# neonnnnn/sparsepoly

Measured on AMD Instinct MI355X. Metric: pcd_epochs_per_sec, higher is better.
Workload: dtype f32; 1 GPU; BASELINE configs[1]: degree=2 n_components=30 regularizer=squaredl12 solver=pcd fit_linear=True fit_lower=explicit on 1000000x100000 CSR nnz=49987865 (~50/row); schedule=colored, parallelism=single GPU, ranks=1, launcher=external, persistent_fallbacks=0

## Files before the change

sparsepoly_amd/csrc/spfm_engine_core.hip:

```cpp
#include "spfm_engine.hip.h"
#include "spfm_linear.hip.h"
#include "spfm_predict.hip.h"
#include "spfm_pbcd.hip.h"

using namespace spfm;

static thread_local std::string g_create_error;

namespace {
struct ncclUniqueId_ {
    char internal[128];
};
enum { ncclSum_ = 0 };
enum { ncclFloat64_ = 8 };
struct Rccl {
    void* lib = nullptr;
    int (*GetUniqueId)(ncclUniqueId_*) = nullptr;
    int (*CommInitRank)(ncclComm_t*, int, ncclUniqueId_, int) = nullptr;
    int (*AllReduce)(const void*, void*, size_t, int, int, ncclComm_t, hipStream_t) = nullptr;
    int (*CommDestroy)(ncclComm_t) = nullptr;
    const char* (*GetErrorString)(int) = nullptr;
    const char* (*GetLastError)(ncclComm_t) = nullptr;
    int (*GetVersion)(int*) = nullptr;
    std::string path;
// ... 1068 lines not shown
int spfm_cd_linear_epoch(spfm_handle h, double alpha, double* viol) {
    SPFM_GUARD(h);
    return h->cd_linear_epoch(alpha, viol);
}

int spfm_pcd_epoch(spfm_handle h, int order_idx, int degree, double beta, double gamma,
                   double eta, const int32_t* indices_component, int n_comp, double* viol) {
    SPFM_GUARD(h);
    return h->pcd_epoch(order_idx, degree, beta, gamma, eta, indices_component, n_comp, viol);
}

int spfm_pbcd_epoch(spfm_handle h, int order_idx, int degree, double beta, double gamma,
                    double eta, double* viol) {
    SPFM_GUARD(h);
    return h->pbcd_epoch(order_idx, degree, beta, gamma, eta, viol);
}

int spfm_host_epoch_begin(spfm_handle h, int order_idx, int degree) {
    SPFM_GUARD(h);
    return h->host_epoch_begin(order_idx, degree);
}
int spfm_host_pass_begin(spfm_handle h, int component) {
    SPFM_GUARD(h);
    return h->host_pass_begin(component);
}
int spfm_host_step_sums(spfm_handle h, int step, double* sums_out) {
    SPFM_GUARD(h);
    return h->host_step(true, step, sums_out, nullptr, nullptr);
}
int spfm_host_step_apply(spfm_handle h, int step, const double* p_new, const double* p_old) {
    SPFM_GUARD(h);
    return h->host_step(false, step, nullptr, p_new, p_old);
}
int spfm_host_epoch_end(spfm_handle h, double* viol) {
    SPFM_GUARD(h);
    return h->host_epoch_end(viol);
}

int spfm_psgd_epoch(spfm_handle h, int degree, double alpha, double beta, double gamma,
                    double eta0, int learning_rate, double power_t, int64_t batch_size,
                    const int32_t* indices_samples, int64_t n_samples, int fit_linear,
                    int64_t* it, double* sum_loss) {
    SPFM_GUARD(h);
    if (h->dist()) {
        h->err = "psgd: several ranks share this handle's communicator -- use spfm_psgd_epoch_sharded";
        return SPFM_ERR_INVALID;
    }
    return h->psgd_epoch(degree, alpha, beta, gamma, eta0, learning_rate, power_t, batch_size,
                         indices_samples, n_samples, 0, fit_linear, it, sum_loss);
}

int spfm_psgd_epoch_sharded(spfm_handle h, int degree, double alpha, double beta, double gamma,
                            double eta0, int learning_rate, double power_t, int64_t batch_size,
                            const int32_t* indices_samples, int64_t n_global, int64_t row_lo,
                            int fit_linear, int64_t* it, double* sum_loss) {
    SPFM_GUARD(h);
    return h->psgd_epoch(degree, alpha, beta, gamma, eta0, learning_rate, power_t, batch_size,
                         indices_samples, n_global, row_lo, fit_linear, it, sum_loss);
}

int spfm_comm_unique_id(char* id128) {
    if (!id128) return SPFM_ERR_INVALID;
    std::string e;
    if (!g_rccl.load(e)) {
        g_create_error = e;
        return SPFM_ERR_RUNTIME;
    }
    ncclUniqueId_ id;
    if (g_rccl.GetUniqueId(&id) != 0) {
        g_create_error = "ncclGetUniqueId failed";
        return SPFM_ERR_RUNTIME;
    }
    std::memcpy(id128, id.internal, 128);
    return SPFM_OK;
}

int spfm_comm_init(spfm_handle h, const char* id128, int n_ranks, int rank) {
    SPFM_GUARD(h);
    if (!id128 || n_ranks < 1 || rank < 0 || rank >= n_ranks) return SPFM_ERR_INVALID;
    if (!g_rccl.load(h->err)) return SPFM_ERR_RUNTIME;
    ncclUniqueId_ id;
    std::memcpy(id.internal, id128, 128);
    (void)hipStreamSynchronize(h->stream);
    const hipError_t stale = h->keep_last_error ? hipSuccess : hipGetLastError();
    int rc = g_rccl.CommInitRank(&h->comm, n_ranks, id, rank);
    if (rc != 0) {
        int ver = 0;
        if (g_rccl.GetVersion) (void)g_rccl.GetVersion(&ver);
        const char* detail = g_rccl.GetLastError ? g_rccl.GetLastError(nullptr) : nullptr;
        h->err = std::string("ncclCommInitRank: ") +
                 (g_rccl.GetErrorString ? g_rccl.GetErrorString(rc) : "error");
        if (detail && *detail) h->err += std::string(" [") + detail + "]";
        h->err += " (librccl " + std::to_string(ver) + " from " + g_rccl.path;
        h->err += std::string("; HIP last error now: ") + hipGetErrorString(hipPeekAtLastError());
        if (stale != hipSuccess)
            h->err += std::string("; cleared before the call: ") + hipGetErrorString(stale);
        h->err += "; set NCCL_DEBUG=INFO for RCCL's own log)";
        h->comm = nullptr;
        return SPFM_ERR_RUNTIME;
    }
    h->n_ranks = n_ranks;
    h->rank = rank;
    h->col_norm_reduced = false;
    h->resident_agreed.clear();
    h->clear_graphs();
    return SPFM_OK;
}

int spfm_comm_init_shm(spfm_handle h, const char* shm_name, int n_ranks, int rank) {
    SPFM_GUARD(h);
    if (!shm_name || n_ranks < 1 || n_ranks > 64 || rank < 0 || rank >= n_ranks)
        return SPFM_ERR_INVALID;
    if (h->comm || h->shm.hdr) {
        h->err = "a communicator is already attached";
        return SPFM_ERR_INVALID;
    }
    using Shm = spfm_engine::ShmComm;
    const size_t bytes = sizeof(Shm::Hdr) + sizeof(double) * Shm::kMaxDoubles * (size_t)n_ranks;
    int fd = shm_open(shm_name, O_RDWR | O_CREAT, 0600);
    if (fd < 0) {
        h->err = std::string("shm_open failed: ") + std::strerror(errno);
        return SPFM_ERR_RUNTIME;
    }
    if (ftruncate(fd, (off_t)bytes) != 0) {
        h->err = std::string("ftruncate failed: ") + std::strerror(errno);
        close(fd);
        return SPFM_ERR_RUNTIME;
    }
    void* p = mmap(nullptr, bytes, PROT_READ | PROT_WRITE, MAP_SHARED, fd, 0);
    close(fd);
    if (p == MAP_FAILED) {
        h->err = std::string("mmap failed: ") + std::strerror(errno);
        return SPFM_ERR_RUNTIME;
    }
    h->shm.hdr = reinterpret_cast<Shm::Hdr*>(p);
    h->shm.slots = reinterpret_cast<double*>(reinterpret_cast<char*>(p) + sizeof(Shm::Hdr));
    h->shm.bytes = bytes;
    h->shm.local_sense = 0;
    h->n_ranks = n_ranks;
    h->rank = rank;
    h->resident_agreed.clear();
    h->col_norm_reduced = false;
    h->clear_graphs();
    return SPFM_OK;
}

int spfm_peer_alloc(spfm_handle h, char* handle64) {
    SPFM_GUARD(h);
    if (!handle64) return SPFM_ERR_INVALID;
    if (!h->peer_own) {
        void* p = nullptr;
        hipError_t ae = hipExtMallocWithFlags(&p, sizeof(double) * spfm_engine::kPeerDoubles,
                                              hipDeviceMallocFinegrained);
        if (ae != hipSuccess) {
            (void)hipGetLastError();
            h->err = std::string("peer slab: fine-grained device memory is not available (") +
                     hipGetErrorString(ae) + "); use the per-step collective";
            return SPFM_ERR_RUNTIME;
        }
        if (hipMemsetAsync(p, 0, sizeof(double) * spfm_engine::kPeerDoubles, h->stream) != hipSuccess ||
            hipStreamSynchronize(h->stream) != hipSuccess) {
            (void)hipFree(p);
            h->err = "peer slab memset failed";
            return SPFM_ERR_RUNTIME;
        }
        h->peer_own = p;
    }
    static_assert(sizeof(hipIpcMemHandle_t) == 64, "IPC handle size");
    hipIpcMemHandle_t ih;
    hipError_t e = hipIpcGetMemHandle(&ih, h->peer_own);
    if (e != hipSuccess) {
        h->err = std::string("hipIpcGetMemHandle: ") + hipGetErrorString(e);
        return SPFM_ERR_RUNTIME;
    }
    std::memcpy(handle64, &ih, 64);
    return SPFM_OK;
}

int spfm_peer_connect(spfm_handle h, int n_ranks, int rank, const char* handles) {
    SPFM_GUARD(h);
    if (!handles || n_ranks < 2 || n_ranks > 8 || rank < 0 || rank >= n_ranks)
        return SPFM_ERR_INVALID;
    if (!h->peer_own) {
        h->err = "spfm_peer_connect: call spfm_peer_alloc first";
        return SPFM_ERR_INVALID;
    }
    if (!h->dist() || h->n_ranks != n_ranks || h->rank != rank) {
        h->err = "spfm_peer_connect: attach the communicator (spfm_comm_init[_shm]) with the "
                 "same ranks first";
        return SPFM_ERR_INVALID;
    }
    h->peer_ptr.assign((size_t)n_ranks, nullptr);
    for (int r = 0; r < n_ranks; ++r) {
        if (r == rank) {
            h->peer_ptr[(size_t)r] = h->peer_own;
            continue;
        }
        hipIpcMemHandle_t ih;
        std::memcpy(&ih, handles + (size_t)r * 64, 64);
        void* p = nullptr;
        hipError_t e = hipIpcOpenMemHandle(&p, ih, hipIpcMemLazyEnablePeerAccess);
        if (e != hipSuccess) {
            h->err = std::string("hipIpcOpenMemHandle: ") + hipGetErrorString(e);
            return SPFM_ERR_RUNTIME;
        }
        h->peer_ptr[(size_t)r] = p;
    }
    std::vector<double*> t1((size_t)n_ranks), t2((size_t)n_ranks);
    for (int r = 0; r < n_ranks; ++r) {
        t1[(size_t)r] = reinterpret_cast<double*>(h->peer_ptr[(size_t)r]) + spfm_engine::kPeerPcdOff;
        t2[(size_t)r] = reinterpret_cast<double*>(h->peer_ptr[(size_t)r]) + spfm_engine::kPeerPbOff;
    }
    if (h->upload(h->peer_tab_pcd, t1.data(), (size_t)n_ranks, 8) ||
        h->upload(h->peer_tab_pb, t2.data(), (size_t)n_ranks, 8) || h->sync()) {
        h->err = "peer table upload failed";
        return SPFM_ERR_RUNTIME;
    }
    {
        DevBuf okb;
        int ok = 0;
        h->peer_generation += 1;
        const unsigned long long word = 0x5350464d00000000ull + (unsigned)h->peer_generation;
        const unsigned long long ticks = 100ull * 1000 * 1000 * 10;
        if (okb.alloc(sizeof(int) * 4) != hipSuccess ||
            hipMemsetAsync(okb.p, 0, sizeof(int) * 4, h->stream) != hipSuccess) {
            h->err = "peer handshake: allocation failed";
            return SPFM_ERR_RUNTIME;
        }
        hipLaunchKernelGGL(peer_probe_kernel, dim3(1), dim3(kWave), 0, h->stream,
                           h->peer_tab_pcd.as<double*>(),
                           spfm_engine::kPeerProbeOff - spfm_engine::kPeerPcdOff, n_ranks, rank,
                           word, ticks, okb.as<int>());
        if (h->download(&ok, okb.p, 1) || h->sync()) {
            h->err = "peer handshake kernel failed";
            return SPFM_ERR_RUNTIME;
        }
        if (!ok) {
            h->err = "peer handshake timed out: a peer's store into this GPU's exchange slab did "
                     "not become visible to a running kernel (use the per-step collective)";
            return SPFM_ERR_RUNTIME;
        }
    }
    h->peer_ready = true;
    h->invalidate(spfm_engine::kInvSchedule | spfm_engine::kInvStreams | spfm_engine::kInvGraphs);
    return SPFM_OK;
}

int spfm_profile_enable(spfm_handle h, int on) {
    if (!h) return SPFM_ERR_INVALID;
    h->prof_on = on != 0;
    return SPFM_OK;
}

int spfm_profile_get(spfm_handle h, int which, double* ms, int64_t* launches, int64_t* nnz) {
    if (!h || which < 0 || which > 4) return SPFM_ERR_INVALID;
    if (ms) *ms = h->prof[which].ms;
    if (launches) *launches = h->prof[which].launches;
    if (nnz) *nnz = h->prof[which].nnz;
    return SPFM_OK;
}

int spfm_profile_reset(spfm_handle h) {
    if (!h) return SPFM_ERR_INVALID;
    for (auto& ps : h->prof) {
        ps.ms = 0;
        ps.launches = 0;
        ps.nnz = 0;
        ps.used = 0;
    }
    return SPFM_OK;
}

#include "spfm_options.inc.h"

int spfm_debug_prb_stamps(spfm_handle h, long long* out, int cap) {
    SPFM_GUARD(h);
    if ((h->pb_dbg & 8) && out && cap >= 8) {
        static unsigned v[16 + 4096];
        if (hipMemcpy(v, h->pb_dbgbuf.p, sizeof v, hipMemcpyDeviceToHost) != hipSuccess)
            return SPFM_ERR_RUNTIME;
        int i = 0;
        for (; i < 16 + 4096 && i < cap; ++i) out[i] = (long long)v[i];
        return i - (i % 16);
    }
    if (h->wide_stamp_on && h->wide_stamps.p && out) {
        const int nv = (int)(h->wide_stamps.bytes / sizeof(long long));
        if (cap < nv) return SPFM_ERR_INVALID;
        if (hipMemcpy(out, h->wide_stamps.p, sizeof(long long) * (size_t)nv,
                      hipMemcpyDeviceToHost) != hipSuccess)
            return SPFM_ERR_RUNTIME;
        return nv;
    }
    if (h->pb_stamp_on && (h->pb_stream_ready || h->pbr_state == 1) && out) {
        const int nv = 16 * (h->pbr_state == 1 ? h->pbr_G : h->pb_stream_G);
        if (cap < nv) return SPFM_ERR_INVALID;
        if (hipMemcpy(out, h->pb_stamps.p, sizeof(long long) * (size_t)nv,
                      hipMemcpyDeviceToHost) != hipSuccess)
            return SPFM_ERR_RUNTIME;
        return nv;
    }
    if (!h->prb_ready || !out) return SPFM_ERR_INVALID;
    const int nval = 16 * h->prb_G;
    if (cap < nval) return SPFM_ERR_INVALID;
    if (hipMemcpy(out, h->prb_stamps.p, sizeof(long long) * (size_t)nval, hipMemcpyDeviceToHost) !=
        hipSuccess)
        return SPFM_ERR_RUNTIME;
    return nval;
}

int spfm_debug_hop_latency(spfm_handle h, int partner, int rounds, double* ns_per_hop,
                           int* xcc_ids ) {
    SPFM_GUARD(h);
    if (partner < 1 || partner > 255 || rounds < 1 || rounds > (1 << 20) || !ns_per_hop)
        return SPFM_ERR_INVALID;
    DevBuf words, info;
    if (words.alloc(sizeof(unsigned long long) * 32) != hipSuccess ||
        info.alloc(sizeof(int) * 4) != hipSuccess)
        return SPFM_ERR_RUNTIME;
    hipEvent_t e0, e1;
    if (hipEventCreate(&e0) != hipSuccess || hipEventCreate(&e1) != hipSuccess)
        return SPFM_ERR_RUNTIME;
    float best = 1e30f;
    int hinfo[4] = {0, 0, 0, 0};
    for (int rep = 0; rep < 3; ++rep) {
        (void)hipMemsetAsync(words.p, 0, sizeof(unsigned long long) * 32, h->stream);
        (void)hipMemsetAsync(info.p, 0, sizeof(int) * 4, h->stream);
        (void)hipEventRecord(e0, h->stream);
        hipLaunchKernelGGL(hop_pingpong_kernel, dim3(partner + 1), dim3(kWave), 0, h->stream,
                           words.as<unsigned long long>(), rounds, partner, info.as<int>());
        (void)hipEventRecord(e1, h->stream);
        if (hipStreamSynchronize(h->stream) != hipSuccess) {
            h->err = "hop_pingpong_kernel failed";
            return SPFM_ERR_RUNTIME;
        }
        float ms = 0.f;
        (void)hipEventElapsedTime(&ms, e0, e1);
        (void)hipMemcpy(hinfo, info.p, sizeof(int) * 4, hipMemcpyDeviceToHost);
        if (hinfo[2] != 0) {
            h->err = "hop latency probe: partner workgroup did not respond";
            (void)hipEventDestroy(e0);
            (void)hipEventDestroy(e1);
            return SPFM_ERR_RUNTIME;
        }
        if (rep > 0 && ms < best) best = ms;
    }
    (void)hipEventDestroy(e0);
    (void)hipEventDestroy(e1);
    *ns_per_hop = (double)best * 1e6 / (2.0 * rounds);
    if (xcc_ids) {
        xcc_ids[0] = hinfo[0];
        xcc_ids[1] = hinfo[1];
    }
    return SPFM_OK;
}

int spfm_debug_exchange_cost(spfm_handle h, int groups, int ncols, int readers_mod, int rounds,
                             double* ns_per_round) {
    SPFM_GUARD(h);
    if (groups < 1 || groups > 256 || ncols < 1 || ncols > 64 || readers_mod == 0 ||
        rounds < 1 || rounds > (1 << 20) || !ns_per_round)
        return SPFM_ERR_INVALID;
    DevBuf slab, abortw;
    const size_t bytes = sizeof(double) * 2 * (2 * (size_t)groups + 2) * 64 * 2;
    if (slab.alloc(bytes) != hipSuccess || abortw.alloc(16) != hipSuccess) return SPFM_ERR_RUNTIME;
    PrbArgs a{};
    a.G = groups;
    a.slab = slab.as<double>();
    a.abort_flag = abortw.as<unsigned>();
    a.spin_max = 1u << 21;
    hipEvent_t e0, e1;
    if (hipEventCreate(&e0) != hipSuccess || hipEventCreate(&e1) != hipSuccess)
        return SPFM_ERR_RUNTIME;
    (void)hipFuncSetAttribute((const void*)exchange_probe_kernel,
                              hipFuncAttributeMaxDynamicSharedMemorySize, (int)h->kPrbLds);
    float best = 1e30f;
    unsigned aborted = 0;
    for (int rep = 0; rep < 3; ++rep) {
        (void)hipMemsetAsync(slab.p, 0, bytes, h->stream);
        (void)hipMemsetAsync(abortw.p, 0, 16, h->stream);
        (void)hipEventRecord(e0, h->stream);
        hipLaunchKernelGGL(exchange_probe_kernel, dim3(h->probe_xcd ? 8 * groups + 64 : groups),
                           dim3(readers_mod == -12 ? 768 : 512),
                           h->probe_xcd ? (size_t)h->probe_lds : (size_t)h->kPrbLds, h->stream, a,
                           rounds, ncols, readers_mod, h->probe_xcd);
        (void)hipEventRecord(e1, h->stream);
        if (hipStreamSynchronize(h->stream) != hipSuccess) {
            h->err = "exchange_probe_kernel failed";
            return SPFM_ERR_RUNTIME;
        }
        float ms = 0.f;
        (void)hipEventElapsedTime(&ms, e0, e1);
        (void)hipMemcpy(&aborted, abortw.p, sizeof(unsigned), hipMemcpyDeviceToHost);
        if (aborted) break;
        if (rep > 0 && ms < best) best = ms;
    }
    (void)hipEventDestroy(e0);
    (void)hipEventDestroy(e1);
    if (aborted) {
        h->err = "exchange probe timed out (workgroups not co-resident?)";
        return SPFM_ERR_RUNTIME;
    }
    *ns_per_round = (double)best * 1e6 / rounds;
    return SPFM_OK;
}

int spfm_debug_stream_probe(spfm_handle h, int64_t* bytes_out) {
    SPFM_GUARD(h);
    return h->debug_stream_probe(bytes_out);
}

int spfm_debug_write_probe(spfm_handle h, int bytes_per_record, int64_t* bytes_out) {
    SPFM_GUARD(h);
    return h->debug_write_probe(bytes_per_record, bytes_out);
}

int spfm_debug_branch_counts(spfm_handle h, unsigned* out8, int reset) {
    SPFM_GUARD(h);
    if (!out8) return SPFM_ERR_INVALID;
    if (hipStreamSynchronize(h->stream) != hipSuccess) return SPFM_ERR_RUNTIME;
    for (int i = 0; i < BR_COUNT; ++i) out8[i] = 0;
    hipError_t (*const units[])(unsigned*, int) = {
        spfm_branch_counts_pcd,       spfm_branch_counts_prb_f32,   spfm_branch_counts_prb_f64,
        spfm_branch_counts_wide,      spfm_branch_counts_pbcd,      spfm_branch_counts_pbprb_f32,
        spfm_branch_counts_pbprb_f64};
    for (auto unit : units)
        if (unit(out8, reset) != hipSuccess) return SPFM_ERR_RUNTIME;
    return SPFM_OK;
}

int spfm_set_use_graph(spfm_handle h, int on) {
    if (!h) return SPFM_ERR_INVALID;
    h->use_graph = on != 0;
    if (!on) h->clear_graphs();
    return SPFM_OK;
}

}
```

sparsepoly_amd/csrc/spfm_engine_prb.inc.h:

```cpp
#include "spfm_engine.hip.h"
#include "spfm_pcd.hip.h"

using namespace spfm;

template <typename T, int LOSS>
int spfm_engine::lin_prb(double alpha) {
    const double mu = loss == SPFM_LOSS_SQUARED ? 1.0 : (loss == SPFM_LOSS_LOGISTIC ? 0.25 : 2.0);
    int rc = ensure_prb<T>();
    if (rc) return rc;
    constexpr bool can_lr = std::is_same<T, float>::value;
    constexpr int LRV = (LOSS == LOSS_SQUARED) ? 1 : 2;
    bool relaxed = false;
    if (relax_candidate()) {
        rc = ensure_relax<T>();
        if (rc) return rc;
        relaxed = relax_state == 1;
    }
    const PrbArgs pa = relaxed ? relax_args() : prb_args();
    int lds_max = 0;
    HIPC(hipDeviceGetAttribute(&lds_max, hipDeviceAttributeMaxSharedMemoryPerBlock, device));
    const size_t lds_lr = sizeof(double) * (kPrbLdsFixed + (relaxed ? kPrbLdsCR : 0)) +
                          (size_t)pa.rows_per * 5 + 16;
    const bool use_lr = can_lr && prb_lds && lds_lr <= (size_t)lds_max && (LRV == 1 || y_pm1);
    const size_t lds_bytes = use_lr ? std::max(lds_lr, kPrbLds) : kPrbLds;
    if constexpr (can_lr) {
        if (use_lr)
            HIPC(hipFuncSetAttribute((const void*)lin_prb_kernel<T, LOSS, LRV>,
                                     hipFuncAttributeMaxDynamicSharedMemorySize,
                                     (int)lds_bytes));
    }
    HIPC(hipFuncSetAttribute((const void*)lin_prb_kernel<T, LOSS, 0>,
                             hipFuncAttributeMaxDynamicSharedMemorySize, (int)kPrbLds));
    hipLaunchKernelGGL(gather_sched_kernel, dim3(cdiv(d, 256)), dim3(256), 0, stream, d,
                       d_desc.as<ColDesc>(), w.as<double>(), prow_old.as<double>());
    HIPC(hipMemsetAsync(prb_slab.p, 0, prb_slab.bytes, stream));
    if (relaxed) HIPC(hipMemsetAsync(r_cslab.p, 0, r_cslab.bytes, stream));
    {
        int prc = peer_clear(kPeerPcdOff, kPeerPbOff);
        if (prc) return prc;
    }
    prof_begin(4, nnz);
    bool launched = false;
    auto launch_cr = [&](auto lr_tag, size_t lds) -> int {
        constexpr int LRc = decltype(lr_tag)::value;
        auto* fn = lin_prb_kernel<T, LOSS, LRc, false, true>;
        HIPC(hipFuncSetAttribute((const void*)fn, hipFuncAttributeMaxDynamicSharedMemorySize,
                                 (int)lds));
        if (!resident_ok((const void*)fn, kPrbThreads, lds, prb_G)) return kNotResident;
        hipLaunchKernelGGL(fn, dim3(launch_groups(prb_G)), dim3(kPrbThreads), lds, stream, pa,
                           r_eval.as<T>(), yy.as<T>(), prow_old.as<double>(),
                           prb_cn.as<double>(), w.as<double>(), alpha, mu,
                           prb_viol.as<double>());
        return SPFM_OK;
    };
    auto launch = [&](auto lr_tag, auto mg_tag, size_t lds) -> int {
        constexpr int LRc = decltype(lr_tag)::value;
        constexpr bool MGc = decltype(mg_tag)::value;
        HIPC(hipFuncSetAttribute((const void*)lin_prb_kernel<T, LOSS, LRc, MGc>,
                                 hipFuncAttributeMaxDynamicSharedMemorySize, (int)lds));
        if (!resident_ok((const void*)lin_prb_kernel<T, LOSS, LRc, MGc>, kPrbThreads, lds, prb_G))
            return kNotResident;
        hipLaunchKernelGGL((lin_prb_kernel<T, LOSS, LRc, MGc>), dim3(launch_groups(prb_G)),
                           dim3(kPrbThreads),
                           lds, stream, pa, prb_eval.as<T>(), yy.as<T>(),
                           prow_old.as<double>(), prb_cn.as<double>(), w.as<double>(), alpha,
                           mu, prb_viol.as<double>());
        return SPFM_OK;
    };
    int lrc = SPFM_OK;
    if (relaxed) {
        launched = true;
        bool done = false;
        if constexpr (can_lr) {
            if (use_lr) {
                lrc = launch_cr(std::integral_constant<int, LRV>{}, lds_bytes);
                done = true;
            }
        }
        if (!done) lrc = launch_cr(std::integral_constant<int, 0>{}, kPrbLds);
    }
    if constexpr (can_lr) {
        if (use_lr && !launched) {
            lrc = pa.n_ranks > 1
                      ? launch(std::integral_constant<int, LRV>{}, std::true_type{}, lds_bytes)
                      : launch(std::integral_constant<int, LRV>{}, std::false_type{}, lds_bytes);
            launched = true;
        }
    }
    if (!launched)
        lrc = pa.n_ranks > 1
                  ? launch(std::integral_constant<int, 0>{}, std::true_type{}, kPrbLds)
                  : launch(std::integral_constant<int, 0>{}, std::false_type{}, kPrbLds);
    if (lrc == kNotResident) prof_cancel(4, nnz);
    if (lrc) return lrc;
    prof_end(4);
    hipLaunchKernelGGL(fold_viol_kernel, dim3(cdiv(d, 256)), dim3(256), 0, stream, d,
                       d_desc.as<ColDesc>(), prb_viol.as<double>(), viol_col.as<double>());
    HIPC(hipGetLastError());
    return SPFM_OK;
}

template <typename T>
int spfm_engine::lin_prb_loss(double alpha) {
    switch (loss) {
        case SPFM_LOSS_SQUARED: return lin_prb<T, LOSS_SQUARED>(alpha);
        case SPFM_LOSS_SQUARED_HINGE: return lin_prb<T, LOSS_SQUARED_HINGE>(alpha);
        default: return lin_prb<T, LOSS_LOGISTIC>(alpha);
    }
}

template <typename T>
int spfm_engine::ensure_prb() {
    if (prb_ready) return SPFM_OK;
    int ncu = 0;
    HIPC(hipDeviceGetAttribute(&ncu, hipDeviceAttributeMultiprocessorCount, device));
    if (prb_G > ncu) prb_G = ncu;
    if (prb_G < 1) prb_G = 1;
    const int nb_ = n_batches();
    std::unique_lock<std::mutex> cache_lock;
    std::string ckey;
    bool hit = false;
    if (scache) {
        ckey = fkey("prb", {}, {(int64_t)sched_hash, prb_G, prb_long, (int64_t)sizeof(T), nb_});
        cache_lock = std::unique_lock<std::mutex>(scache->mu);
        for (auto& e : scache->prb)
            if (e->key == ckey) {
                prb_sp.share(e->sp);
                prb_erow.share(e->erow);
                prb_eval.share(e->eval);
                prb_lmask.share(e->lmask);
                prb_has_long = e->has_long;
                stream_device_used = 2;
                hit = true;
                break;
            }
    }
    if (!hit) {
        int rc = build_prb_stream<T>(nb_);
        if (rc) return rc;
        if (scache) {
            auto e = std::make_unique<StreamCache::Prb>();
            e->key = ckey;
            e->sp.share(prb_sp);
            e->erow.share(prb_erow);
            e->eval.share(prb_eval);
            e->lmask.share(prb_lmask);
            e->has_long = prb_has_long;
            scache->prb.insert(scache->prb.begin(), std::move(e));
            if (scache->prb.size() > StreamCache::kKeep) scache->prb.pop_back();
        }
    }
    if (cache_lock.owns_lock()) cache_lock.unlock();
    HIPC(prb_slab.alloc(sizeof(double) * 2 * ((size_t)prb_G + 1) * 64 * 2));
    HIPC(prb_abort.alloc(sizeof(unsigned) * 4));
    HIPC(prow_old.alloc(sizeof(double) * (size_t)d));
    HIPC(prb_viol.alloc(sizeof(double) * (size_t)d));
    HIPC(prb_cn.alloc(sizeof(double) * (size_t)d));
    HIPC(prb_stamps.alloc(sizeof(long long) * 16 * (size_t)prb_G));
    HIPC(hipMemsetAsync(prb_stamps.p, 0, prb_stamps.bytes, stream));
    HIPC(hipMemsetAsync(prb_abort.p, 0, sizeof(unsigned) * 4, stream));
    HIPC(hipMemsetAsync(prb_slab.p, 0, prb_slab.bytes, stream));
    hipLaunchKernelGGL(gather_sched_kernel, dim3(cdiv(d, 256)), dim3(256), 0, stream, d,
                       d_desc.as<ColDesc>(), col_norm.as<double>(), prb_cn.as<double>());
    HIPC(hipGetLastError());
    HIPC(hipStreamSynchronize(stream));
    prb_ready = true;
    return SPFM_OK;
}

template <typename T>
int spfm_engine::build_prb_stream(int nb_) {
    const size_t nsp = (size_t)prb_G * nb_ * 65 + 1;
    DevBuf d_src;
    HIPC(d_src.alloc(sizeof(int32_t) * (size_t)(nnz > 0 ? nnz : 1)));
    HIPC(prb_sp.alloc(sizeof(int32_t) * nsp));
    HIPC(prb_lmask.alloc(sizeof(uint32_t) * (size_t)prb_G * nb_ * 2));
    stream_device_used = 0;
    if (stream_device && nnz >= (1 << 20)) {
        int hl = 0;
        const hipError_t e = device_rowblock_stream(
            n, d, nnz, prb_G, nb_, prb_long, d_order.as<int32_t>(), d_bptr.as<int32_t>(),
            cptr.as<int64_t>(), cidx.as<int32_t>(), nullptr, prb_sp.as<int32_t>(),
            d_src.as<int32_t>(), prb_lmask.as<uint32_t>(), &hl, nullptr, stream);
        if (e == hipSuccess) {
            prb_has_long = hl;
            stream_device_used = 1;
        } else {
            (void)hipGetLastError();
        }
    }
    std::vector<int32_t> sp, src;
    std::vector<uint32_t> lmask;
    if (!stream_device_used) {
        build_rowblock_stream(n, h_cptr.data(), h_cidx.data(), order, batch_ptr, prb_G,
                              prb_long, sp, src, lmask, nullptr);
        prb_has_long = 0;
        for (uint32_t m : lmask) prb_has_long |= (m != 0u);
        SPFM_TRY(upload_to(prb_lmask.p, lmask.data(), lmask.size()));
    }
    HIPC(prb_erow.alloc(sizeof(int32_t) * (size_t)(nnz > 0 ? nnz : 1)));
    HIPC(prb_eval.alloc(sizeof(T) * (size_t)(nnz > 0 ? nnz : 1)));
    if (!stream_device_used)
        SPFM_TRY(upload_to(prb_sp.p, sp.data(), sp.size()));
    if (nnz > 0) {
        if (!stream_device_used)
            SPFM_TRY(upload_to(d_src.p, src.data(), (size_t)nnz));
        hipLaunchKernelGGL((prb_gather_kernel<T>), dim3(cdiv(nnz, 256)), dim3(256), 0, stream,
                           nnz, d_src.as<int32_t>(), cidx.as<int32_t>(), cval.as<T>(),
                           prb_erow.as<int32_t>(), prb_eval.as<T>());
        HIPC(hipGetLastError());
    }
    HIPC(hipStreamSynchronize(stream));
    return SPFM_OK;
}

template <typename T>
int spfm_engine::ensure_relax() {
    if (relax_state != 0) return SPFM_OK;
    relax_state = -1;
    int rc = ensure_prb<T>();
    if (rc) return rc;
    std::vector<int32_t> cf_ptr, cf_row, cf_qq, sp, src;
    std::vector<int64_t> cf_ia, cf_ib;
    std::vector<int16_t> clist;
    std::vector<uint8_t> skip;
    std::vector<uint32_t> lmask;
    schedule_relax(n, d, h_cptr.data(), h_cidx.data(), order.data(), 64, 64, r_batch_ptr, cf_ptr,
                   cf_row, cf_qq, cf_ia, cf_ib, clist, skip);
    const int nbr = (int)r_batch_ptr.size() - 1;
    if ((double)nbr > 0.6 * (double)n_batches()) return SPFM_OK;
    DevBuf d_src;
    HIPC(r_bptr.alloc(sizeof(int32_t) * r_batch_ptr.size()));
    SPFM_TRY(upload_to(r_bptr.p, r_batch_ptr.data(), r_batch_ptr.size()));
    const size_t nsp_r = (size_t)prb_G * nbr * 65 + 1;
    bool dev_stream = false;
    size_t ne = 0;
    if (stream_device && nnz >= (1 << 20)) {
        DevBuf d_skip;
        HIPC(d_skip.alloc((size_t)nnz));
        SPFM_TRY(upload_to(d_skip.p, skip.data(), (size_t)nnz));
        HIPC(d_src.alloc(sizeof(int32_t) * (size_t)nnz));
        HIPC(r_sp.alloc(sizeof(int32_t) * nsp_r));
        HIPC(r_lmask.alloc(sizeof(uint32_t) * (size_t)prb_G * nbr * 2));
        int hl = 0;
        int64_t tot = 0;
        const hipError_t e = device_rowblock_stream(
            n, d, nnz, prb_G, nbr, prb_long, d_order.as<int32_t>(), r_bptr.as<int32_t>(),
            cptr.as<int64_t>(), cidx.as<int32_t>(), d_skip.as<uint8_t>(), r_sp.as<int32_t>(),
            d_src.as<int32_t>(), r_lmask.as<uint32_t>(), &hl, &tot, stream);
        if (e == hipSuccess) {
            relax_has_long = hl;
            ne = (size_t)tot;
            dev_stream = true;
        } else {
            (void)hipGetLastError();
        }
    }
    if (!dev_stream) {
        build_rowblock_stream(n, h_cptr.data(), h_cidx.data(), order, r_batch_ptr, prb_G,
                              prb_long, sp, src, lmask, skip.data());
        relax_has_long = 0;
        for (uint32_t m : lmask) relax_has_long |= (m != 0u);
        ne = src.size();
    }
    const size_t ncf = cf_row.size();
    std::vector<PrbConf<T>> hcf(ncf ? ncf : 1);
    {
        std::vector<T> hv((size_t)(nnz > 0 ? nnz : 1));
        SPFM_TRY(download(hv.data(), cval.p, (size_t)nnz));
        HIPC(hipStreamSynchronize(stream));
        for (size_t c = 0; c < ncf; ++c) {
            hcf[c].row = cf_row[c];
            hcf[c].qq = cf_qq[c];
            hcf[c].xa = hv[(size_t)cf_ia[c]];
            hcf[c].xb = hv[(size_t)cf_ib[c]];
        }
    }
    if (!dev_stream) {
        HIPC(d_src.alloc(sizeof(int32_t) * (ne ? ne : 1)));
        HIPC(r_sp.alloc(sizeof(int32_t) * sp.size()));
        HIPC(r_lmask.alloc(sizeof(uint32_t) * lmask.size()));
    }
    HIPC(r_erow.alloc(sizeof(int32_t) * (ne ? ne : 1)));
    HIPC(r_eval.alloc(sizeof(T) * (ne ? ne : 1)));
    HIPC(r_cfptr.alloc(sizeof(int32_t) * cf_ptr.size()));
    HIPC(r_cf.alloc(sizeof(PrbConf<T>) * hcf.size()));
    HIPC(r_clist.alloc(sizeof(int16_t) * clist.size() + 16));
    HIPC(r_cslab.alloc(sizeof(double) * 2 * 64 * 8));
    if (!dev_stream) {
        SPFM_TRY(upload_to(r_sp.p, sp.data(), sp.size()));
        SPFM_TRY(upload_to(r_lmask.p, lmask.data(), lmask.size()));
    }
    SPFM_TRY(upload_to(r_cfptr.p, cf_ptr.data(), cf_ptr.size()));
    SPFM_TRY(upload_to(r_cf.p, hcf.data(), hcf.size()));
    SPFM_TRY(upload_to(r_clist.p, clist.data(), clist.size()));
    if (ne > 0) {
        if (!dev_stream)
            SPFM_TRY(upload_to(d_src.p, src.data(), ne));
        hipLaunchKernelGGL((prb_gather_kernel<T>), dim3(cdiv((int64_t)ne, 256)), dim3(256), 0,
                           stream, (int64_t)ne, d_src.as<int32_t>(), cidx.as<int32_t>(),
                           cval.as<T>(), r_erow.as<int32_t>(), r_eval.as<T>());
        HIPC(hipGetLastError());
    }
    HIPC(hipStreamSynchronize(stream));
    relax_state = 1;
    return SPFM_OK;
}

template <typename T, int M, int LOSS>
int spfm_engine::pcd_pass_prb(int order_idx, double beta, double gamma, double eta) {
    const double mu = loss == SPFM_LOSS_SQUARED ? 1.0 : (loss == SPFM_LOSS_LOGISTIC ? 0.25 : 2.0);
    int rc = ensure_prb<T>();
    if (rc) return rc;
    double* Po = P.as<double>() + (size_t)order_idx * k * d;
    Ctl* c = ctl.as<Ctl>();
    double* cb = cache.as<double>();
    constexpr bool can_lr = std::is_same<T, float>::value && Kind<M>::AS <= 2;
    constexpr int LRV = (LOSS == LOSS_SQUARED) ? 1 : 2;
    constexpr bool can_stamp = std::is_same<T, float>::value && M == 2 && LOSS == LOSS_SQUARED;
    constexpr bool can_stamp3 = std::is_same<T, float>::value && M == 3 && LOSS == LOSS_SQUARED;
    if (prb_stamp_on && !((can_stamp && prb_lds) || (can_stamp3 && !prb_lds)))
        FAIL(SPFM_ERR_UNSUPPORTED,
             "prb_stamps: built for float storage, squared loss and degree 2 with prb_lds=1 "
             "or degree 3 with prb_lds=0 only");
    bool relaxed = false;
    if constexpr (M == 2 || M == 3) {
        if (relax_candidate() && !prb_stamp_on) {
            rc = ensure_relax<T>();
            if (rc) return rc;
            relaxed = relax_state == 1;
        }
    }
    PrbArgs pa = relaxed ? relax_args() : prb_args();
    constexpr bool can_pk = std::is_same<T, float>::value && M == 3;
    bool packed = false;
    if (prb_stamp_on && pa.n_ranks > 1)
        FAIL(SPFM_ERR_UNSUPPORTED,
             "prb_stamps: the timer instantiation has no cross-GPU stage (single rank only)");
    int lds_max = 0;
    HIPC(hipDeviceGetAttribute(&lds_max, hipDeviceAttributeMaxSharedMemoryPerBlock, device));
    const size_t lds_lr = sizeof(double) * (kPrbLdsFixed + (relaxed ? kPrbLdsCR : 0)) +
                          (size_t)pa.rows_per * (4 * Kind<M>::AS + (LRV == 1 ? 4 : 5)) + 16;
    const bool use_lr = can_lr && prb_lds && lds_lr <= (size_t)lds_max &&
                        (LRV == 1 || y_pm1);
    const size_t lds_bytes = use_lr ? std::max(lds_lr, kPrbLds) : kPrbLds;
    prb_lds_active = use_lr ? LRV : 0;
    hipLaunchKernelGGL(begin_pass_kernel, dim3(1), dim3(64), 0, stream, c,
                       comp_order.as<int32_t>(), lams.as<double>());
    if (reg != SPFM_REG_L1) {
        hipLaunchKernelGGL((pcd_compute_cache_kernel<M>), dim3(kCacheBlocks), dim3(kBlock), 0,
                           stream, c, Po, d, reg, partial.as<double>());
        hipLaunchKernelGGL((pcd_cache_combine_kernel<M>), dim3(1), dim3(64), 0, stream, reg,
                           kCacheBlocks, partial.as<double>(), cb);
    }
    hipLaunchKernelGGL(snapshot_row_kernel, dim3(cdiv(d, 256)), dim3(256), 0, stream, c, Po, d,
                       d_desc.as<ColDesc>(), prow_old.as<double>());
    HIPC(hipMemsetAsync(prb_slab.p, 0, prb_slab.bytes, stream));
    if (relaxed) HIPC(hipMemsetAsync(r_cslab.p, 0, r_cslab.bytes, stream));
    if constexpr (can_pk) {
        if (!use_lr && !prb_stamp_on && prb_pack) {
            HIPC(prb_rec.alloc(sizeof(float) * 4 * (size_t)n));
            pa.rec = prb_rec.p;
            hipLaunchKernelGGL(prb_pack3_kernel, dim3(cdiv(n, 256)), dim3(256), 0, stream, c, n,
                               (size_t)n * 2, yy.as<float>(), A.as<float>(),
                               prb_rec.as<float4>());
            packed = true;
        }
    }
    {
        int prc = peer_clear(kPeerPcdOff, kPeerPbOff);
        if (prc) return prc;
    }
    prof_begin(0, nnz);
    auto go = [&](auto lr_tag, auto stamp_tag, auto reg_tag) -> int {
        constexpr int LRc = decltype(lr_tag)::value;
        constexpr bool STc = decltype(stamp_tag)::value;
        constexpr int RGc = decltype(reg_tag)::value;
        const size_t lds = (LRc == 1 || LRc == 2) ? lds_bytes : kPrbLds;
        auto launch = [&](auto mg_tag) -> int {
            constexpr bool MGc = decltype(mg_tag)::value;
            HIPC(hipFuncSetAttribute(
                (const void*)pcd_prb_kernel<T, M, LOSS, LRc, STc, RGc, MGc>,
                hipFuncAttributeMaxDynamicSharedMemorySize, (int)lds));
            if (!resident_ok((const void*)pcd_prb_kernel<T, M, LOSS, LRc, STc, RGc, MGc>,
                             kPrbThreads, lds, prb_G))
                return kNotResident;
            hipLaunchKernelGGL((pcd_prb_kernel<T, M, LOSS, LRc, STc, RGc, MGc>),
                               dim3(launch_groups(prb_G)), dim3(kPrbThreads), lds, stream, c, pa, prb_eval.as<T>(),
                               A.as<T>(), (size_t)n * Kind<M>::AS, yy.as<T>(),
                               prow_old.as<double>(), Po, d, reg, cb, mu, beta, gamma, eta,
                               prb_viol.as<double>());
            return SPFM_OK;
        };
        if constexpr (STc) {
            return launch(std::false_type{});
        } else {
            return pa.n_ranks > 1 ? launch(std::true_type{}) : launch(std::false_type{});
        }
    };
    using std::integral_constant;
    int lrc = SPFM_OK;
    bool launched = false;
    if constexpr (M == 2 || M == 3) {
        if (relaxed) {
            auto launch_cr = [&](auto lr_tag) -> int {
                constexpr int LRc = decltype(lr_tag)::value;
                const size_t lds = (LRc == 1 || LRc == 2) ? lds_bytes : kPrbLds;
                auto* fn = pcd_prb_kernel<T, M, LOSS, LRc, false, -1, false, true>;
                HIPC(hipFuncSetAttribute((const void*)fn,
                                         hipFuncAttributeMaxDynamicSharedMemorySize, (int)lds));
                if (!resident_ok((const void*)fn, kPrbThreads, lds, prb_G)) return kNotResident;
                hipLaunchKernelGGL(fn, dim3(launch_groups(prb_G)), dim3(kPrbThreads), lds, stream,
                                   c, pa, r_eval.as<T>(), A.as<T>(), (size_t)n * Kind<M>::AS,
                                   yy.as<T>(), prow_old.as<double>(), Po, d, reg, cb, mu, beta,
                                   gamma, eta, prb_viol.as<double>());
                return SPFM_OK;
            };
            launched = true;
            bool done = false;
            if constexpr (can_lr) {
                if (use_lr) {
                    lrc = launch_cr(integral_constant<int, LRV>{});
                    done = true;
                }
            }
            if constexpr (can_pk) {
                if (!done && packed) {
                    lrc = launch_cr(integral_constant<int, 3>{});
                    done = true;
                }
            }
            if (!done) lrc = launch_cr(integral_constant<int, 0>{});
        }
    }
    if constexpr (can_lr) {
        if (use_lr && !launched) {
            launched = true;
            if constexpr (can_stamp) {
                if (prb_stamp_on)
                    lrc = go(integral_constant<int, LRV>{}, std::true_type{},
                             integral_constant<int, -1>{});
            }
            if (!prb_stamp_on) {
                if (reg == SPFM_REG_L1)
                    lrc = go(integral_constant<int, LRV>{}, std::false_type{},
                             integral_constant<int, REG_L1>{});
                else if (reg == SPFM_REG_OMEGATI)
                    lrc = go(integral_constant<int, LRV>{}, std::false_type{},
                             integral_constant<int, REG_OMEGATI>{});
                else if constexpr (M == 2)
                    lrc = go(integral_constant<int, LRV>{}, std::false_type{},
                             integral_constant<int, REG_SQL12>{});
                else
                    lrc = go(integral_constant<int, LRV>{}, std::false_type{},
                             integral_constant<int, -1>{});
            }
        }
    }
    if constexpr (can_pk) {
        if (!launched && packed) {
            launched = true;
// ... 61 lines not shown
```

sparsepoly_amd/csrc/spfm_pcd.hip.h:

```cpp
#pragma once
#include "spfm_common.hip.h"

namespace spfm {


template <typename T, int M>
__global__ __launch_bounds__(kBlock) void pcd_precompute_all_kernel(
    int64_t n, int k, const int64_t* __restrict__ rptr, const int32_t* __restrict__ ridx,
    const T* __restrict__ rval, const double* __restrict__ Pt, T* __restrict__ A_all) {
    constexpr int R = 32;
    constexpr int RP = R + 1;
    extern __shared__ __attribute__((aligned(16))) unsigned char pre_lds[];
    T* tile = reinterpret_cast<T*>(pre_lds);
    const int tid = threadIdx.x, lane = tid & 63, wave = tid >> 6;
    for (int64_t tile0 = (int64_t)blockIdx.x * R; tile0 < n; tile0 += (int64_t)gridDim.x * R) {
        for (int s0 = 0; s0 < k; s0 += kWave) {
            const int s = s0 + lane;
            const bool sv = s < k;
            for (int r = wave; r < R; r += kBlock / kWave) {
                const int64_t i = tile0 + r;
                if (i >= n) break;
                constexpr int NA = (M == 0) ? 2 : M;
                double a[NA];
                a[0] = 1.0;
// ... 373 lines not shown
            double r;
            {
                const double dc2 = c10 - a_i;
                const double m0 = p_i - s_i * (c20 - dc2 * a_i);
                r = (m0 > 0) ? m0 : 0.0;
            }
            bool fixed = false;
            unsigned long long negl = 0ull;
            double be1 = 0.0, be2 = 0.0;
            for (int round = 0; round < 8 && !fixed; ++round) {
                const double d1 = r - a_i;
                double al1 = 1.0;
                be1 = d1;
                affine_scan_inclusive(al1, be1, lane);
                const double c1b = affine_before(al1, be1, c10, lane);
                const double dc2 = c1b - a_i;
                double al2 = 1.0;
                be2 = dc2 * d1;
                affine_scan_inclusive(al2, be2, lane);
                const double c2b = affine_before(al2, be2, c20, lane);
                const double dc3 = c2b - dc2 * a_i;
                const double m = p_i - s_i * dc3;
                const double rn = (m > 0) ? m : 0.0;
                negl = __ballot(act && ((__double2hiint(dc2) | __double2hiint(dc3)) < 0));
                fixed = __ballot(__double_as_longlong(rn) != __double_as_longlong(r)) == 0ull;
                r = rn;
            }
            if (fixed && negl == 0ull) {
                cache[1] = c10 + readlane_d(be1, 63);
                cache[2] = c20 + readlane_d(be2, 63);
                return sg * (act ? r : 0.0);
            }
        }
        if constexpr (M > 2) {
            {
                const bool in = lane <= last;
                double* my = sc + lane * 4;
                my[0] = in ? ab : 0.0;
                my[1] = in ? st : 0.0;
                my[2] = in ? apin : 0.0;
            }
            asm volatile("s_waitcnt lgkmcnt(0)" ::: "memory");
            double c[M + 1];
#pragma unroll
            for (int t = 0; t <= M; ++t) c[t] = cache[t];
            unsigned neg = 0u;
            const int nblk = (last + 4) >> 2;
            auto sweep = [&](auto clip_tag) __attribute__((always_inline)) {
                constexpr bool CLIP = decltype(clip_tag)::value;
                double na[4], ns[4], np[4];
#pragma unroll
                for (int u = 0; u < 4; ++u) {
                    na[u] = sc[u * 4];
                    ns[u] = sc[u * 4 + 1];
                    np[u] = sc[u * 4 + 2];
                }
                for (int blk = 0; blk < nblk; ++blk) {
                    double ca[4], cs[4], cp[4];
                    double* nx = sc + (blk + 1) * 16;
#pragma unroll
                    for (int u = 0; u < 4; ++u) {
                        ca[u] = na[u];
                        cs[u] = ns[u];
                        cp[u] = np[u];
                        na[u] = nx[u * 4];
                        ns[u] = nx[u * 4 + 1];
                        np[u] = nx[u * 4 + 2];
                    }
#pragma unroll
                    for (int u = 0; u < 4; ++u) {
                        const double ai = ca[u], si = cs[u], pi = cp[u];
                        double dc[M + 2];
                        dc[1] = 1.0;
#pragma unroll
                        for (int deg = 2; deg <= M; ++deg) {
                            double v = c[deg - 1];
                            v -= dc[deg - 1] * ai;
                            if constexpr (CLIP) {
                                dc[deg] = (v < 0) ? 0.0 : v;
                            } else {
                                neg |= (unsigned)__double2hiint(v);
                                dc[deg] = v;
                            }
                        }
                        const double m = pi - si * dc[M];
                        const double r = (m > 0) ? m : 0.0;
#pragma unroll
                        for (int deg = 1; deg < M; ++deg) c[deg] = dc[deg + 1] + dc[deg] * r;
                        sc[(blk * 4 + u) * 4 + 3] = r;
                    }
                }
            };
            if (lane == 0) sweep(std::false_type{});
            if (__builtin_amdgcn_readfirstlane((int)neg) < 0) {
                count_branch(BR_OMEGATI_CLIP, lane);
#pragma unroll
                for (int t = 0; t <= M; ++t) c[t] = cache[t];
                if (lane == 0) sweep(std::true_type{});
            }
#pragma unroll
            for (int t = 1; t < M; ++t) cache[t] = readlane_d(c[t], 0);
            asm volatile("s_waitcnt lgkmcnt(0)" ::: "memory");
            mine = (lane <= last) ? sc[lane * 4 + 3] : 0.0;
        }
        return sg * mine;
    }
}


template <int M>
__device__ __forceinline__ double pcd_chain_waves(int reg, int lane, int wave, int ncols, bool valid,
                                                  double p_old, double g, double h, double lam,
                                                  double mu, double beta, double gamma, double eta,
                                                  double (&cache)[M + 1], double* sh_map,
                                                  int* sh_bad) {
    static_assert(M == 2, "wide steps: degree 2");
    double pin = 0.0, st = 0.0;
    if (valid) {
        double inv = h * mu;
        inv += beta;
        double upd = g * lam;
        upd += beta * p_old;
        const double rinv = recip_nr(inv);
        upd *= rinv;
        pin = p_old - eta * upd;
        st = (eta * gamma) * rinv;
    }
    if (reg == REG_L1) {
        const double sg = (pin > 0) ? 1.0 : ((pin < 0) ? -1.0 : 0.0);
        const double m = fabs(pin) - st;
        return sg * (m > 0.0 ? m : 0.0);
    }
    const bool sq = reg == REG_SQL12;
    const int nw = (ncols + 63) >> 6;
    const int last = min(64, ncols - 64 * wave) - 1;
    const bool act = valid && lane <= last;
    const double ab = fabs(p_old);
    double app, tt, sg;
    if (sq) {
        const double rden = recip_nr(1 + 2 * st);
        const double pp = pin * rden;
        app = fabs(pp);
        tt = (2 * st) * rden;
        sg = (pp > 0) ? 1.0 : -1.0;
    } else {
        app = fabs(pin);
        tt = st;
        sg = (pin > 0) ? 1.0 : -1.0;
    }
    const int ci = sq ? 0 : 1;
    const double c0 = cache[ci];
    bool pos = sq ? true : ((c0 - ab) >= 0);
    bool nz = (app - tt * (pos ? (c0 - ab) : 0.0)) > 0;
    double al = 1.0, be = 0.0, m = 0.0;
    auto scan = [&]() __attribute__((always_inline)) {
        if (!act) {
            al = 1.0;
            be = 0.0;
        } else if (!pos) {
            al = 0.0;
            be = app;
        } else if (nz) {
            al = 1.0 - tt;
            be = app - al * ab;
        } else {
            al = 1.0;
            be = -ab;
        }
        affine_scan_inclusive(al, be, lane);
    };
    scan();
    bool dirty = true;
    double mA[8], mB[8];
#pragma unroll
    for (int w = 0; w < 8; ++w) {
        mA[w] = 1.0;
        mB[w] = 0.0;
    }
    for (int gr = 0; gr < 3 * kWave; ++gr) {
        if (dirty && lane == 0) {
            sh_map[wave * 2] = last >= 0 ? readlane_d(al, last >= 0 ? last : 0) : 1.0;
            sh_map[wave * 2 + 1] = last >= 0 ? readlane_d(be, last >= 0 ? last : 0) : 0.0;
        }
        if (wave == 0 && lane == 0) {
            if (gr == 0) sh_bad[0] = sh_bad[1] = sh_bad[2] = 0;
            else sh_bad[(gr + 1) % 3] = 0;
        }
        asm volatile("s_waitcnt lgkmcnt(0)\n\ts_barrier" ::: "memory");
#pragma unroll
        for (int w = 0; w < 8; ++w) {
            mA[w] = sh_map[w * 2];
            mB[w] = sh_map[w * 2 + 1];
        }
        double c_in = c0;
#pragma unroll
        for (int w = 0; w < 7; ++w)
            if (w < wave) c_in = mA[w] * c_in + mB[w];
        bool changed = false;
        for (int lr = 0; lr <= kWave; ++lr) {
            const double cb = affine_before(al, be, c_in, lane);
            const double v = cb - ab;
            const bool pos2 = sq ? true : !(v < 0);
            const double u = pos2 ? v : 0.0;
            m = sq ? fma(-tt, u, app) : (app - tt * u);
            const bool nz2 = m > 0;
            const unsigned long long bad =
                __ballot(act && ((pos2 != pos) || (pos2 && (nz2 != nz))));
            pos = pos2;
            nz = nz2;
            if (bad == 0ull) break;
            changed = true;
            scan();
        }
        dirty = changed;
        if (changed && lane == 0) sh_bad[gr % 3] = 1;
        asm volatile("s_waitcnt lgkmcnt(0)\n\ts_barrier" ::: "memory");
        if (sh_bad[gr % 3] == 0) break;
    }
    if (!sq && __ballot(act && !pos) != 0ull) count_branch(BR_OMEGATI_CLIP, lane);
    double c_end = c0;
#pragma unroll
    for (int w = 0; w < 8; ++w)
        if (w < nw) c_end = mA[w] * c_end + mB[w];
    cache[ci] = c_end;
    const double r = sq ? ((act && nz) ? m : 0.0) : (act ? ((m > 0) ? m : 0.0) : 0.0);
    return sg * r;
}

template <int M>
__global__ __launch_bounds__(kWave) void pcd_chain_kernel(
    const Ctl* __restrict__ ctl, const ColDesc* __restrict__ desc, int ncols,
    double* __restrict__ P, int d, const double* __restrict__ part,
    const double* __restrict__ pold, int reg, const double* __restrict__ cache_in,
    double* __restrict__ cache_out, double mu, double beta, double gamma, double eta,
    double* __restrict__ delta, double* __restrict__ viol_col) {
    __shared__ double sh_chain[(kWave + 4) * 4];
    const int lane = threadIdx.x;
    const double lam = ctl->lam;
    double* ps = P + (size_t)ctl->s * d;
    double cache[M + 1];
#pragma unroll
    for (int t = 0; t <= M; ++t) cache[t] = cache_in[t];
    for (int base = 0; base < ncols; base += kWave) {
        const int q = base + lane;
        const bool valid = q < ncols;
        const int cnt = min(kWave, ncols - base);
        double p_old = 0.0, g = 0.0, h = 0.0;
        int j = 0;
        if (valid) {
            j = desc[q].j;
            p_old = pold[q];
            g = part[2 * q];
            h = part[2 * q + 1];
        }
        const double res =
            pcd_chain_lanes<M>(reg, lane, cnt - 1, valid, p_old, g, h, lam, mu, beta, gamma, eta,
                               cache, sh_chain);
        if (valid) {
            const double dl = p_old - res;
            ps[j] = res;
            delta[q] = dl;
            viol_col[j] += fabs(dl);
        }
    }
    if (lane == 0) {
#pragma unroll
        for (int t = 0; t <= M; ++t) cache_out[t] = cache[t];
    }
}


template <typename T, int M>
__device__ __forceinline__ void pcd_sync_entry(size_t i, double x, double p_old, double upd,
                                               double lam, T* __restrict__ A,
                                               T* __restrict__ yy) {
    if constexpr (M == 0) {
        const double a0 = (double)A[i];
        double yh = (double)yy[2 * i];
        yh -= lam * a0;
        double a1 = a0 / (1.0 + x * p_old);
        a1 *= 1.0 + x * (p_old - upd);
        yh += lam * a1;
        A[i] = (T)a1;
        yy[2 * i] = (T)yh;
        return;
    }
    double dprev = x;
#pragma unroll
    for (int t = 1; t < M; ++t) {
        const size_t at = i * (M - 1) + (t - 1);
        const double a = (double)A[at];
        const double dcur = x * (a - p_old * dprev);
        A[at] = (T)(a - upd * dprev);
        dprev = dcur;
    }
    const double yh = (double)yy[2 * i];
    yy[2 * i] = (T)(yh - lam * upd * dprev);
}

template <typename T, int M>
__device__ __forceinline__ void pcd_sync_entry_lds(int il, double x, double p_old, double upd,
                                                   double lam, T* lds_a, T* lds_r) {
    constexpr int AS = Kind<M>::AS;
    double yh = (double)lds_r[il];
    if constexpr (M == 0) {
        const double a0 = (double)lds_a[il];
        yh -= lam * a0;
        double a1 = a0 / (1.0 + x * p_old);
        a1 *= 1.0 + x * (p_old - upd);
        yh += lam * a1;
        lds_a[il] = (T)a1;
        lds_r[il] = (T)yh;
    } else {
        double dprev = x;
#pragma unroll
        for (int t = 0; t < AS; ++t) {
            const double a = (double)lds_a[il * AS + t];
            const double dcur = x * (a - p_old * dprev);
            lds_a[il * AS + t] = (T)(a - upd * dprev);
            dprev = dcur;
        }
        lds_r[il] = (T)(yh - lam * upd * dprev);
    }
}

template <typename T, int M>
__global__ __launch_bounds__(kBlock) void pcd_sync_kernel(
    const Ctl* __restrict__ ctl, const ColDesc* __restrict__ desc,
    const int32_t* __restrict__ cidx, const T* __restrict__ cval, T* __restrict__ A_all,
    size_t a_stride, T* __restrict__ yy , const double* __restrict__ delta,
    const double* __restrict__ pold) {
    const int q = blockIdx.x;
    const double upd = delta[q];
    if (upd == 0.0) return;
    T* __restrict__ A = A_all + (size_t)ctl->s * a_stride;
    const double p_old = pold[q];
    const double lam = ctl->lam;
    const ColDesc cd = desc[q];
    const int64_t b = cd.start, e = cd.start + cd.len;
    for (int64_t ii = b + threadIdx.x; ii < e; ii += kBlock)
        pcd_sync_entry<T, M>((size_t)cidx[ii], (double)cval[ii], p_old, upd, lam, A, yy);
}

template <typename T, int M>
__global__ __launch_bounds__(kBlock) void pcd_chain_sync_kernel(
    const Ctl* __restrict__ ctl, const ColDesc* __restrict__ desc, int ncols,
    double* __restrict__ P, int d, const double* __restrict__ part,
    const double* __restrict__ pold, int reg, const double* __restrict__ cache_in,
    double* __restrict__ cache_out, double mu, double beta, double gamma, double eta,
    const int32_t* __restrict__ cidx, const T* __restrict__ cval, T* __restrict__ A_all,
    size_t a_stride, T* __restrict__ yy, double* __restrict__ viol_col) {
    __shared__ double sh[2];
    __shared__ double sh_chain[(kWave + 4) * 4];
    T* __restrict__ A = A_all + (size_t)ctl->s * a_stride;
    constexpr int PF = 2;
    const int q = blockIdx.x;
    const int tid = threadIdx.x, lane = tid & 63, wave = tid >> 6;
    const ColDesc cd = desc[q];
    const double lam = ctl->lam;
    int ri[PF];
    double rx[PF];
    bool rv[PF];
#pragma unroll
    for (int u = 0; u < PF; ++u) {
        const int off = tid + u * kBlock;
        rv[u] = off < cd.len;
        ri[u] = rv[u] ? cidx[cd.start + off] : 0;
        rx[u] = rv[u] ? (double)cval[cd.start + off] : 0.0;
    }
    if (wave == 0) {
        const bool valid = lane < ncols;
        double p_old = 0.0, g = 0.0, h = 0.0;
        if (valid) {
            p_old = pold[lane];
            g = part[2 * lane];
            h = part[2 * lane + 1];
        }
        double cache[M + 1];
#pragma unroll
        for (int t = 0; t <= M; ++t) cache[t] = cache_in[t];
        const double res = pcd_chain_lanes<M>(reg, lane, q, valid, p_old, g, h, lam, mu, beta,
                                              gamma, eta, cache, sh_chain);
        if (lane == q) {
            const double dl = p_old - res;
            P[(size_t)ctl->s * d + cd.j] = res;
            viol_col[cd.j] += fabs(dl);
            sh[0] = dl;
            sh[1] = p_old;
        }
        if (q == ncols - 1 && lane == 0) {
#pragma unroll
            for (int t = 0; t <= M; ++t) cache_out[t] = cache[t];
        }
    }
    __syncthreads();
    const double upd = sh[0];
    if (upd == 0.0) return;
    const double p_old = sh[1];
#pragma unroll
    for (int u = 0; u < PF; ++u)
        if (rv[u]) pcd_sync_entry<T, M>((size_t)ri[u], rx[u], p_old, upd, lam, A, yy);
    for (int64_t ii = cd.start + tid + PF * kBlock; ii < cd.start + cd.len; ii += kBlock)
        pcd_sync_entry<T, M>((size_t)cidx[ii], (double)cval[ii], p_old, upd, lam, A, yy);
}


}
```

sparsepoly_amd/csrc/spfm_prb.hip.h:

```cpp
#pragma once
#include "spfm_common.hip.h"
#include "spfm_pcd.hip.h"

namespace spfm {


struct PrbArgs {
    int G;
    int nb;
    const int32_t* bptr;
    const ColDesc* desc;
    const int32_t* sp;
    const uint32_t* lmask;
    int has_long;
    const int32_t* erow;
    double* slab;
    int rows_per;
    int n_rows;
    unsigned* abort_flag;
    unsigned spin_max;
    long long* stamps;
    int n_ranks, rank;
    double* const* xslab;
    const int32_t* cf_ptr;
    const void* cf;
    const int16_t* clist;
    double* cslab;
    void* rec;
};

template <typename T>
struct __attribute__((aligned(8))) PrbConf {
    int32_t row;
    int32_t qq;
    T xa, xb;
};


__device__ __forceinline__ void st_agent(double* p, double v) {
    __hip_atomic_store(reinterpret_cast<unsigned long long*>(p),
                       (unsigned long long)__double_as_longlong(v), __ATOMIC_RELAXED,
                       __HIP_MEMORY_SCOPE_AGENT);
}
__device__ __forceinline__ double ld_agent(const double* p) {
    const unsigned long long u =
        __hip_atomic_load(reinterpret_cast<const unsigned long long*>(p), __ATOMIC_RELAXED,
                          __HIP_MEMORY_SCOPE_AGENT);
    return __longlong_as_double((long long)u);
}

__device__ __forceinline__ unsigned long long prb_tag(int b) {
    return (unsigned long long)(((b >> 1) % 3) + 1);
}
__device__ __forceinline__ void prb_store_granule(double* p, double v, unsigned long long tag) {
    const unsigned long long u =
        ((unsigned long long)__double_as_longlong(v) & ~3ull) | tag;
    __hip_atomic_store(reinterpret_cast<unsigned long long*>(p), u, __ATOMIC_RELAXED,
                       __HIP_MEMORY_SCOPE_AGENT);
}
__device__ __forceinline__ unsigned long long prb_load_granule(const double* p) {
    return __hip_atomic_load(reinterpret_cast<const unsigned long long*>(p), __ATOMIC_RELAXED,
                             __HIP_MEMORY_SCOPE_AGENT);
}

__device__ __forceinline__ void prb_store_granule_l2(double* p, double v, unsigned long long tag) {
    const unsigned long long u =
        ((unsigned long long)__double_as_longlong(v) & ~3ull) | tag;
    asm volatile("global_store_dwordx2 %0, %1, off" ::"v"(p), "v"(u) : "memory");
}

__device__ __forceinline__ void prb_store_granule_sys(double* p, double v, unsigned long long tag) {
    const unsigned long long u =
        ((unsigned long long)__double_as_longlong(v) & ~3ull) | tag;
    __hip_atomic_store(reinterpret_cast<unsigned long long*>(p), u, __ATOMIC_RELAXED,
                       __HIP_MEMORY_SCOPE_SYSTEM);
}
__device__ __forceinline__ unsigned long long prb_load_granule_sys(const double* p) {
    return __hip_atomic_load(reinterpret_cast<const unsigned long long*>(p), __ATOMIC_RELAXED,
                             __HIP_MEMORY_SCOPE_SYSTEM);
}

template <int NV>
__device__ __forceinline__ bool prb_cross_gpu(const PrbArgs& a, int g, int b, int lane,
                                              double* tot) {
    const unsigned long long tag = prb_tag(b);
    const size_t par_off = (size_t)(b & 1) * a.n_ranks * 64 * 2;
    if (g == 0) {
        for (int rr = 0; rr < a.n_ranks; ++rr) {
            double* dst = a.xslab[rr] + par_off + ((size_t)a.rank * 64 + lane) * 2;
#pragma unroll
            for (int v = 0; v < NV; ++v) prb_store_granule_sys(dst + v, tot[v], tag);
        }
    }
    const double* mine = a.xslab[a.rank] + par_off + (size_t)lane * 2;
    double acc[NV];
#pragma unroll
    for (int v = 0; v < NV; ++v) acc[v] = 0.0;
    for (int rr = 0; rr < a.n_ranks; ++rr) {
        unsigned long long t[NV];
        unsigned spins = 0;
        for (;;) {
            bool all = true;
#pragma unroll
            for (int v = 0; v < NV; ++v) {
                t[v] = prb_load_granule_sys(mine + (size_t)rr * 64 * 2 + v);
                all = all && ((t[v] & 3ull) == tag);
            }
            if (all) break;
            if ((++spins & 63u) == 0) {
                if (__hip_atomic_load(a.abort_flag, __ATOMIC_RELAXED, __HIP_MEMORY_SCOPE_AGENT) ||
                    spins > a.spin_max) {
                    __hip_atomic_store(a.abort_flag, 1u, __ATOMIC_RELAXED,
                                       __HIP_MEMORY_SCOPE_AGENT);
                    return false;
                }
            }
        }
#pragma unroll
        for (int v = 0; v < NV; ++v) acc[v] += __longlong_as_double((long long)(t[v] & ~3ull));
    }
#pragma unroll
    for (int v = 0; v < NV; ++v) tot[v] = acc[v];
    return true;
}

typedef unsigned __attribute__((ext_vector_type(4))) prb_u4;

__device__ __forceinline__ void prb_load_pairs8(const double* const* p, prb_u4* r) {
    asm volatile(
        "global_load_dwordx4 %0, %8, off sc1\n\t"
        "global_load_dwordx4 %1, %9, off sc1\n\t"
        "global_load_dwordx4 %2, %10, off sc1\n\t"
        "global_load_dwordx4 %3, %11, off sc1\n\t"
        "global_load_dwordx4 %4, %12, off sc1\n\t"
        "global_load_dwordx4 %5, %13, off sc1\n\t"
        "global_load_dwordx4 %6, %14, off sc1\n\t"
        "global_load_dwordx4 %7, %15, off sc1\n\t"
        "s_waitcnt vmcnt(0)"
        : "=&v"(r[0]), "=&v"(r[1]), "=&v"(r[2]), "=&v"(r[3]), "=&v"(r[4]), "=&v"(r[5]),
          "=&v"(r[6]), "=&v"(r[7])
        : "v"(p[0]), "v"(p[1]), "v"(p[2]), "v"(p[3]), "v"(p[4]), "v"(p[5]), "v"(p[6]), "v"(p[7])
        : "memory");
}

template <int NV>
__device__ __forceinline__ bool prb_collect_quarter(const PrbArgs& a, int b, int w, int lane,
                                                    int ncols, double* out ,
                                                    int nparts = 4) {
    const double* slab = a.slab + (size_t)(b & 1) * a.G * 64 * 2;
    const unsigned long long tag = prb_tag(b);
    const int g0 = (a.G * w) / nparts, g1 = (a.G * (w + 1)) / nparts;
    double tot[NV];
#pragma unroll
    for (int v = 0; v < NV; ++v) tot[v] = 0.0;
    bool ok = true;
    if (lane < ncols) {
        const double* sl = slab + (size_t)lane * 2;
        constexpr int GU = 8;
        for (int gg = g0; gg < g1; gg += GU) {
            unsigned long long t[GU][NV];
            unsigned spins = 0;
            for (;;) {
                bool all = true;
                if constexpr (NV == 2) {
                    const double* ptr[GU];
                    prb_u4 r[GU];
#pragma unroll
                    for (int u = 0; u < GU; ++u)
                        ptr[u] = sl + (size_t)((gg + u < g1) ? gg + u : g1 - 1) * 128;
                    prb_load_pairs8(ptr, r);
#pragma unroll
                    for (int u = 0; u < GU; ++u) {
                        t[u][0] = ((unsigned long long)r[u].y << 32) | r[u].x;
                        t[u][1] = ((unsigned long long)r[u].w << 32) | r[u].z;
                        all = all && ((t[u][0] & 3ull) == tag) && ((t[u][1] & 3ull) == tag);
                    }
                } else {
#pragma unroll
                    for (int u = 0; u < GU; ++u)
#pragma unroll
                        for (int v = 0; v < NV; ++v) {
                            const bool in = gg + u < g1;
                            t[u][v] = in ? prb_load_granule(sl + (size_t)(gg + u) * 128 + v) : tag;
                            all = all && ((t[u][v] & 3ull) == tag);
                        }
                }
                if (all) break;
                if ((++spins & 63u) == 0) {
                    if (__hip_atomic_load(a.abort_flag, __ATOMIC_RELAXED,
                                          __HIP_MEMORY_SCOPE_AGENT) ||
                        spins > a.spin_max) {
                        __hip_atomic_store(a.abort_flag, 1u, __ATOMIC_RELAXED,
                                           __HIP_MEMORY_SCOPE_AGENT);
                        ok = false;
                        break;
                    }
                }
            }
            if (!ok) break;
#pragma unroll
            for (int u = 0; u < GU; ++u)
#pragma unroll
                for (int v = 0; v < NV; ++v)
                    if (gg + u < g1) tot[v] += __longlong_as_double((long long)(t[u][v] & ~3ull));
        }
    }
#pragma unroll
    for (int v = 0; v < NV; ++v) out[((size_t)w * 64 + lane) * 2 + v] = tot[v];
    return ok;
}

constexpr int PRB_PF = 4;
constexpr int kPrbLong = 48;
template <typename T>
struct PrbEntries {
    int e0, e1;
    int row[PRB_PF];
    T x[PRB_PF];
};

__device__ __forceinline__ void prb_load_sp(const PrbArgs& a, int g, int b, int slot, int ncols,
                                            int& e0, int& e1, unsigned long long& lmask) {
    e0 = 0;
    e1 = 0;
    lmask = 0ull;
    const int32_t* spb = a.sp + ((size_t)g * a.nb + b) * 65;
    if (a.has_long) {
        const uint32_t* lm = a.lmask + ((size_t)g * a.nb + b) * 2;
        lmask = ((unsigned long long)lm[1] << 32) | (unsigned long long)lm[0];
        if (slot < ncols && !((lmask >> slot) & 1ull)) {
            e0 = spb[slot];
            e1 = spb[slot + 1];
        }
    } else if (slot < ncols) {
        e0 = spb[slot];
        e1 = spb[slot + 1];
    }
}

__device__ __forceinline__ int nth_set_bit(unsigned long long m, int q) {
    for (int t = 0; t < q; ++t) m &= m - 1;
    return __builtin_ctzll(m);
}

template <typename T>
__device__ __forceinline__ void prb_load_entries(const PrbArgs& a, const T* __restrict__ eval,
                                                 int e0, int e1, int sub, PrbEntries<T>& en,
                                                 int pad_row = 0) {
    en.e0 = e0;
    en.e1 = e1;
#pragma unroll
    for (int u = 0; u < PRB_PF; ++u) {
        const int e = e0 + sub + 4 * u;
        const bool v = e < e1;
        en.row[u] = v ? a.erow[e] : pad_row;
        en.x[u] = v ? eval[e] : (T)0;
    }
}

constexpr int kPrbThreads = 512;
constexpr int kPrbParts = 8;
constexpr int kPrbLdsFixed = 2560;

template <int NV>
__device__ __forceinline__ bool prb_poll(const PrbArgs& a, const double* p, unsigned long long tag,
                                         double* out);

__device__ __forceinline__ void pcd_sync_entry_rec(size_t i, double x, double p_old, double upd,
                                                   double lam, float4* __restrict__ rec) {
    const float4 r = rec[i];
    const double a1 = (double)r.z, a2 = (double)r.w;
    const double d1 = x * (a1 - p_old * x);
    const double d2 = x * (a2 - p_old * d1);
    float4 o;
    o.x = (float)((double)r.x - lam * upd * d2);
    o.y = r.y;
    o.z = (float)(a1 - upd * x);
    o.w = (float)(a2 - upd * d1);
    rec[i] = o;
}

static __global__ void prb_pack3_kernel(const Ctl* __restrict__ ctl, int64_t n, size_t a_stride,
                                 const float* __restrict__ yy, const float* __restrict__ A_all,
                                 float4* __restrict__ rec) {
    const int64_t i = (int64_t)blockIdx.x * blockDim.x + threadIdx.x;
    if (i < n) {
        const float* A = A_all + (size_t)ctl->s * a_stride;
        float4 r;
        r.x = yy[2 * i];
        r.y = yy[2 * i + 1];
        r.z = A[2 * i];
        r.w = A[2 * i + 1];
        rec[i] = r;
    }
}
static __global__ void prb_unpack3_kernel(const Ctl* __restrict__ ctl, int64_t n, size_t a_stride,
                                   const float4* __restrict__ rec, float* __restrict__ yy,
                                   float* __restrict__ A_all) {
    const int64_t i = (int64_t)blockIdx.x * blockDim.x + threadIdx.x;
    if (i < n) {
        float* A = A_all + (size_t)ctl->s * a_stride;
        const float4 r = rec[i];
        yy[2 * i] = r.x;
        A[2 * i] = r.z;
        A[2 * i + 1] = r.w;
    }
}

constexpr int kPrbLdsCR = 256;
template <typename T, int M, int LOSS, int LR, bool STAMP = false, int REGC = -1, bool MG = false,
          bool CR = false>
__global__ __launch_bounds__(kPrbThreads) void pcd_prb_kernel(
    const Ctl* __restrict__ ctl, PrbArgs a, const T* __restrict__ eval, T* __restrict__ A_all,
    size_t a_stride, T* __restrict__ yy, const double* __restrict__ pold_sched,
    double* __restrict__ P, int d, int reg, const double* __restrict__ cache_in, double mu,
    double beta, double gamma, double eta, double* __restrict__ viol_pos) {
    T* __restrict__ A = A_all + (size_t)ctl->s * a_stride;
    extern __shared__ __attribute__((aligned(16))) double dyn_lds[];
    double* sh_delta = dyn_lds + 128;
    double* sh_pold = dyn_lds + 192;
    double* sh_chain = dyn_lds + 256;
    double* sh_quart = dyn_lds + 1536;
    int* sh_ok = reinterpret_cast<int*>(dyn_lds + 768);
    int* sh_go = reinterpret_cast<int*>(dyn_lds + 770);
    const typename Vec2<T>::type* yy2 = reinterpret_cast<const typename Vec2<T>::type*>(yy);
    const int g = blockIdx.x;
    const int tid = threadIdx.x, lane = tid & 63, wave = tid >> 6;
    const bool control = wave == 0;
    const bool worker = wave >= 1 && wave <= 4;
    const int part = worker ? wave - 1 : (control ? 4 : wave);
    const int wt = tid - 64;
    const int slot = worker ? (wt >> 2) : 64, sub = wt & 3;
    const int s = ctl->s;
    const double lam = ctl->lam;
    double* ps = P + (size_t)s * d;
    double cache[M + 1];
#pragma unroll
    for (int t = 0; t <= M; ++t) cache[t] = cache_in[t];

    double* sh_long = dyn_lds + 1024;
    constexpr bool LDSR = (LR == 1 || LR == 2);
    constexpr bool PK = (LR == 3);
    static_assert(!LDSR || (Kind<M>::AS <= 2 && sizeof(T) == 4 &&
                            (LR == 2 || LOSS == LOSS_SQUARED)),
                  "LDS-resident rows: float storage, one or two cache values per row");
    static_assert(!PK || (sizeof(T) == 4 && Kind<M>::AS == 2),
                  "packed row records: float storage, two cache values per row");
    float4* __restrict__ rec = reinterpret_cast<float4*>(a.rec);
    constexpr int AS = Kind<M>::AS;
    static_assert(!CR || (M >= 2 && !MG && !STAMP), "relaxed runs: degree >= 2, single GPU");
    constexpr int CSN = 2 + Kind<M>::AS;
    constexpr int CSS = 8;
    const int row0 = LDSR ? g * a.rows_per : 0;
    double* sh_ce = dyn_lds + kPrbLdsFixed;
    double* sh_cv = sh_ce + 128;
    T* lds_a = reinterpret_cast<T*>(dyn_lds + kPrbLdsFixed + (CR ? kPrbLdsCR : 0));
    T* lds_r = lds_a + (size_t)a.rows_per * AS;
    unsigned char* lds_s = reinterpret_cast<unsigned char*>(lds_r + a.rows_per);
    if constexpr (LDSR) {
        const int nr = min(a.rows_per, a.n_rows - row0);
        for (int il = tid; il < nr; il += kPrbThreads) {
            const typename Vec2<T>::type yv = yy2[(size_t)(row0 + il)];
#pragma unroll
            for (int t = 0; t < AS; ++t) lds_a[il * AS + t] = A[(size_t)(row0 + il) * AS + t];
            if constexpr (LR == 1) {
                lds_r[il] = (T)((double)yv.x - (double)yv.y);
            } else {
                lds_r[il] = yv.x;
                lds_s[il] = yv.y > (T)0 ? 1 : 0;
            }
        }
        __syncthreads();
    }
    PrbEntries<T> cur, nxt;
    int c0 = a.bptr[0], c1 = a.bptr[1];
    int c2 = (a.nb > 1) ? a.bptr[2] : c1;
    int c3 = (a.nb > 2) ? a.bptr[3] : c2;
    unsigned long long lm0 = 0ull, lm1 = 0ull;
    {
        int e0, e1;
        prb_load_sp(a, g, 0, slot, c1 - c0, e0, e1, lm0);
        prb_load_entries<T>(a, eval, e0, e1, sub, cur, row0);
    }
    int ne0 = 0, ne1 = 0;
    if (a.nb > 1) prb_load_sp(a, g, 1, slot, c2 - c1, ne0, ne1, lm1);
    double p_slot = (slot < c1 - c0) ? pold_sched[c0 + slot] : 0.0;
    if (tid == 0) {
        *sh_ok = 1;
        *sh_go = 0;
    }
    int cp0 = 0, cp1 = 0, cp2 = 0, cp3 = 0;
    PrbConf<T> cfc, cfn;
    cfc.row = cfn.row = 0;
    cfc.qq = cfn.qq = 0;
    cfc.xa = cfc.xb = cfn.xa = cfn.xb = (T)0;
    prb_u4 clq = {~0u, ~0u, ~0u, ~0u}, clqn = {~0u, ~0u, ~0u, ~0u};
    if constexpr (CR) {
        if (control) {
            const PrbConf<T>* cfa = reinterpret_cast<const PrbConf<T>*>(a.cf);
            cp0 = a.cf_ptr[0];
            cp1 = a.cf_ptr[min(1, a.nb)];
            cp2 = a.cf_ptr[min(2, a.nb)];
            cp3 = a.cf_ptr[min(3, a.nb)];
            if (lane < cp1 - cp0) cfc = cfa[cp0 + lane];
            if (lane < c1 - c0)
                clq = reinterpret_cast<const prb_u4*>(a.clist)[c0 + lane];
        }
    }
    long long acc[8] = {0, 0, 0, 0, 0, 0, 0, 0};
    long long tprev = STAMP ? clock64() : 0;
#define PRB_STAMP(k)                        \
    if constexpr (STAMP) {                  \
        if (tid == 0) {                     \
            const long long tn = clock64(); \
            acc[k] += tn - tprev;           \
            tprev = tn;                     \
        }                                   \
    }
#define PRB_HSTAMP(k)                       \
    if constexpr (STAMP) {                  \
        if (tid == 320) {                   \
            const long long tn = clock64(); \
            acc[k] += tn - tprev;           \
            tprev = tn;                     \
        }                                   \
    }
#define PRB_WSTAMP(k)                       \
    if constexpr (STAMP) {                  \
        if (tid == 64) {                    \
            const long long tn = clock64(); \
            acc[k] += tn - tprev;           \
            tprev = tn;                     \
        }                                   \
    }

    for (int b = 0; b < a.nb; ++b) {
        const int ncols = c1 - c0;
        const int c4 = (b + 4 <= a.nb) ? a.bptr[b + 4] : c3;
        __builtin_amdgcn_s_waitcnt(0x0F70);
        double av[PRB_PF][AS];
        double yh[PRB_PF], yt[PRB_PF], dlast[PRB_PF];
        double pl = 0.0;
        int jl = 0;
        double cst[CSN];
#pragma unroll
        for (int t = 0; t < CSN; ++t) cst[t] = 0.0;
        if (control) {
            if (lane < ncols) {
                pl = pold_sched[c0 + lane];
                if (g == 0) jl = a.desc[c0 + lane].j;
            }
            if constexpr (CR) {
                const int nc = cp1 - cp0, ncw = max(nc, cp3 - cp2);
                const unsigned long long ctag = prb_tag(b);
                double* cs = a.cslab + ((size_t)(b & 1) * 64 + lane) * CSS;
                if (lane < nc) {
                    const int i = cfc.row;
                    if (i / a.rows_per == g) {
                        double st[CSN];
                        if constexpr (LDSR) {
                            st[0] = (double)lds_r[i - row0];
                            st[1] = (LR == 1) ? 0.0 : (lds_s[i - row0] ? 1.0 : -1.0);
#pragma unroll
                            for (int t = 0; t < AS; ++t) st[2 + t] = (double)lds_a[(i - row0) * AS + t];
                        } else if constexpr (PK) {
                            const float4 r = rec[(size_t)i];
                            st[0] = (double)r.x;
                            st[1] = (double)r.y;
                            st[2] = (double)r.z;
                            st[2 + AS - 1] = (double)r.w;
                        } else {
                            const typename Vec2<T>::type yv = yy2[(size_t)i];
                            st[0] = (double)yv.x;
                            st[1] = (double)yv.y;
#pragma unroll
                            for (int t = 0; t < AS; ++t) st[2 + t] = (double)A[(size_t)i * AS + t];
                        }
#pragma unroll
                        for (int t = 0; t < CSN; ++t) prb_store_granule(cs + t, st[t], ctag);
                    }
                } else if (lane < ncw && (lane % a.G) == g) {
#pragma unroll
                    for (int t = 0; t < CSN; ++t) prb_store_granule(cs + t, 0.0, ctag);
                }
            }
        } else if (worker) {
#pragma unroll
            for (int u = 0; u < PRB_PF; ++u) {
                if constexpr (LDSR) {
                    const int il = cur.row[u] - row0;
                    yh[u] = (double)lds_r[il];
                    yt[u] = (LR == 1) ? 0.0 : (lds_s[il] ? 1.0 : -1.0);
#pragma unroll
                    for (int t = 0; t < AS; ++t) av[u][t] = (double)lds_a[il * AS + t];
                } else if constexpr (PK) {
                    const float4 r = rec[(size_t)cur.row[u]];
                    yh[u] = (double)r.x;
                    yt[u] = (double)r.y;
                    av[u][0] = (double)r.z;
                    av[u][AS - 1] = (double)r.w;
                } else {
                    const size_t i = (size_t)cur.row[u];
                    const typename Vec2<T>::type yv = yy2[i];
                    yh[u] = (double)yv.x;
                    yt[u] = (double)yv.y;
#pragma unroll
                    for (int t = 0; t < AS; ++t) av[u][t] = (double)A[i * AS + t];
                }
            }
            double ag = 0.0, ah = 0.0;
#pragma unroll
            for (int u = 0; u < PRB_PF; ++u) {
                const double dprev = grad_factor<M>(av[u], (double)cur.x[u], p_slot);
                dlast[u] = dprev;
                const double dl = dloss_dev(LOSS, yh[u], yt[u]);
                const bool v = cur.e0 + sub + 4 * u < cur.e1;
                ag += v ? dl * dprev : 0.0;
                ah += v ? dprev * dprev : 0.0;
            }
            for (int e = cur.e0 + sub + 4 * PRB_PF; e < cur.e1; e += 4) {
                const int i = a.erow[e];
                const double x = (double)eval[e];
                double a1[AS], y0, y1;
                if constexpr (LDSR) {
                    y0 = (double)lds_r[i - row0];
                    y1 = (LR == 1) ? 0.0 : (lds_s[i - row0] ? 1.0 : -1.0);
#pragma unroll
                    for (int t = 0; t < AS; ++t) a1[t] = (double)lds_a[(i - row0) * AS + t];
                } else if constexpr (PK) {
                    const float4 r = rec[(size_t)i];
                    y0 = (double)r.x;
                    y1 = (double)r.y;
                    a1[0] = (double)r.z;
                    a1[AS - 1] = (double)r.w;
                } else {
                    const typename Vec2<T>::type yv = yy2[i];
                    y0 = (double)yv.x;
                    y1 = (double)yv.y;
#pragma unroll
                    for (int t = 0; t < AS; ++t) a1[t] = (double)A[(size_t)i * AS + t];
                }
                const double dprev = grad_factor<M>(a1, x, p_slot);
                ag += dloss_dev(LOSS, y0, y1) * dprev;
                ah += dprev * dprev;
            }
            ag += dpp_move_d<0xB1, 0xf>(0.0, ag);
            ah += dpp_move_d<0xB1, 0xf>(0.0, ah);
            ag += dpp_move_d<0x4E, 0xf>(0.0, ag);
            ah += dpp_move_d<0x4E, 0xf>(0.0, ah);
            PRB_WSTAMP(0)
            if (sub == 0 && !((lm0 >> slot) & 1ull)) {
                double* sl = a.slab + (size_t)(b & 1) * a.G * 64 * 2 + ((size_t)g * 64 + slot) * 2;
                const unsigned long long tag = prb_tag(b);
                prb_store_granule(sl, ag, tag);
                prb_store_granule(sl + 1, ah, tag);
            }
        }
        const unsigned long long lmu =
            ((unsigned long long)__builtin_amdgcn_readfirstlane((int)(lm0 >> 32)) << 32) |
            (unsigned)__builtin_amdgcn_readfirstlane((int)lm0);
        if (lmu != 0ull) {
            const int32_t* spb = a.sp + ((size_t)g * a.nb + b) * 65;
            int qi = 0;
            for (unsigned long long mm = lmu; mm != 0ull; mm &= mm - 1, ++qi) {
                const int q = __builtin_ctzll(mm);
                if (worker) {
                    const int le0 = spb[q], le1 = spb[q + 1];
                    const double pq = pold_sched[c0 + q];
                    double lg = 0.0, lh = 0.0;
                    for (int e = le0 + wt; e < le1; e += 256) {
                        const int i = a.erow[e];
                        const double x = (double)eval[e];
                        double a1[Kind<M>::AS], y0, y1;
                        if constexpr (LDSR) {
                            y0 = (double)lds_r[i - row0];
                            y1 = (LR == 1) ? 0.0 : (lds_s[i - row0] ? 1.0 : -1.0);
#pragma unroll
                            for (int t = 0; t < Kind<M>::AS; ++t)
                                a1[t] = (double)lds_a[(i - row0) * Kind<M>::AS + t];
                        } else if constexpr (PK) {
                            const float4 r = rec[(size_t)i];
                            y0 = (double)r.x;
                            y1 = (double)r.y;
                            a1[0] = (double)r.z;
                            a1[Kind<M>::AS - 1] = (double)r.w;
                        } else {
                            const typename Vec2<T>::type yv = yy2[i];
                            y0 = (double)yv.x;
                            y1 = (double)yv.y;
#pragma unroll
                            for (int t = 0; t < Kind<M>::AS; ++t)
                                a1[t] = (double)A[(size_t)i * Kind<M>::AS + t];
                        }
                        const double dprev = grad_factor<M>(a1, x, pq);
                        lg += dloss_dev(LOSS, y0, y1) * dprev;
                        lh += dprev * dprev;
                    }
                    lg = wave_sum(lg);
                    lh = wave_sum(lh);
                    if (lane == 0) {
                        sh_long[(qi * 4 + (wave - 1)) * 2] = lg;
                        sh_long[(qi * 4 + (wave - 1)) * 2 + 1] = lh;
                    }
                }
            }
            __syncthreads();
            if (worker && wt < qi) {
                const int q = nth_set_bit(lmu, wt);
                double tg = 0.0, th = 0.0;
                for (int w4 = 0; w4 < 4; ++w4) {
                    tg += sh_long[(wt * 4 + w4) * 2];
                    th += sh_long[(wt * 4 + w4) * 2 + 1];
                }
                double* sl = a.slab + (size_t)(b & 1) * a.G * 64 * 2 + ((size_t)g * 64 + q) * 2;
                const unsigned long long tag = prb_tag(b);
                prb_store_granule(sl, tg, tag);
                prb_store_granule(sl + 1, th, tag);
            }
        }
        PRB_STAMP(0)
        double p_next = 0.0;
        int n2e0 = 0, n2e1 = 0;
        unsigned long long lm2 = 0ull;
        if (b + 2 < a.nb) prb_load_sp(a, g, b + 2, slot, c3 - c2, n2e0, n2e1, lm2);
        if (worker) {
            PRB_WSTAMP(1)
            if (tid == 64 + 255)
                __hip_atomic_store(sh_go, b + 1, __ATOMIC_RELAXED, __HIP_MEMORY_SCOPE_WORKGROUP);
            if (LDSR && b + 1 < a.nb) {
                prb_load_entries<T>(a, eval, ne0, ne1, sub, nxt, row0);
                if (slot < c2 - c1) p_next = pold_sched[c1 + slot];
            }
            {
                const bool ok =
                    prb_collect_quarter<2>(a, b, part, lane, ncols, sh_quart, kPrbParts);
                if (!ok) *sh_ok = 0;
            }
            PRB_WSTAMP(2)
            if (!LDSR && b + 1 < a.nb) {
                prb_load_entries<T>(a, eval, ne0, ne1, sub, nxt, row0);
                if (slot < c2 - c1) p_next = pold_sched[c1 + slot];
            }
        } else {
            unsigned spins = 0;
            while (__hip_atomic_load(sh_go, __ATOMIC_RELAXED, __HIP_MEMORY_SCOPE_WORKGROUP) <
                       b + 1 &&
                   ++spins < (1u << 24))
                __builtin_amdgcn_s_sleep(1);
            PRB_HSTAMP(1)
            const bool ok = prb_collect_quarter<2>(a, b, part, lane, ncols, sh_quart, kPrbParts);
            if (!ok) *sh_ok = 0;
            PRB_HSTAMP(2)
            if constexpr (CR) {
                if (control) {
                    if (lane < cp1 - cp0) {
                        if (!prb_poll<CSN>(a, a.cslab + ((size_t)(b & 1) * 64 + lane) * CSS,
                                           prb_tag(b), cst))
                            *sh_ok = 0;
                    }
                    const PrbConf<T>* cfa = reinterpret_cast<const PrbConf<T>*>(a.cf);
                    if (lane < cp2 - cp1) cfn = cfa[cp1 + lane];
                    clqn = prb_u4{~0u, ~0u, ~0u, ~0u};
                    if (lane < c2 - c1) clqn = reinterpret_cast<const prb_u4*>(a.clist)[c1 + lane];
                }
            }
        }
        PRB_WSTAMP(3)
        asm volatile("s_waitcnt lgkmcnt(0)\n\ts_barrier" ::: "memory");
        if (!*sh_ok) break;
        PRB_STAMP(3)
        PRB_HSTAMP(7)
        PRB_WSTAMP(4)
        if (control) {
            double tot[2];
#pragma unroll
            for (int v = 0; v < 2; ++v) {
                tot[v] = sh_quart[lane * 2 + v];
#pragma unroll
                for (int w = 1; w < kPrbParts; ++w) tot[v] += sh_quart[(w * 64 + lane) * 2 + v];
            }
            if constexpr (MG) {
                if (!prb_cross_gpu<2>(a, g, b, lane, tot)) *sh_ok = 0;
            }
            const bool valid = lane < ncols;
            bool serial = false;
            if constexpr (CR) serial = (cp1 - cp0) > 0;
            if (!serial) {
                const double res = pcd_chain_lanes<M>(REGC >= 0 ? REGC : reg, lane, ncols - 1, valid,
                                                      pl, tot[0], tot[1], lam, mu, beta, gamma, eta,
                                                      cache, sh_chain);
                const double dl = valid ? (pl - res) : 0.0;
                sh_delta[lane] = dl;
                sh_pold[lane] = pl;
                if (g == 0 && valid) {
                    ps[jl] = res;
                    viol_pos[c0 + lane] = fabs(dl);
                }
            }
            if constexpr (CR) {
                if (serial) {
                    const int nc = cp1 - cp0;
                    const int qa = cfc.qq & 0xff, qb = cfc.qq >> 8;
                    const double xa = (double)cfc.xa, xb = (double)cfc.xb;
                    sh_pold[lane] = pl;
                    sh_delta[lane] = 0.0;
                    asm volatile("s_waitcnt lgkmcnt(0)" ::: "memory");
                    __builtin_amdgcn_wave_barrier();
                    double da[AS + 1], pb = 0.0;
#pragma unroll
                    for (int t = 0; t <= AS; ++t) da[t] = 0.0;
                    if (lane < nc) {
                        const double pa = sh_pold[qa];
                        pb = sh_pold[qb];
                        da[0] = xa;
#pragma unroll
                        for (int t = 1; t <= AS; ++t) da[t] = xa * (cst[1 + t] - pa * da[t - 1]);
                        sh_ce[lane * 2] = dloss_dev(LOSS, cst[0], cst[1]) * da[AS];
                        sh_ce[lane * 2 + 1] = da[AS] * da[AS];
                    }
                    auto after_a = [&](double Da, double* a1, double& y0n) __attribute__((always_inline)) {
#pragma unroll
                        for (int t = 0; t < AS; ++t) a1[t] = (double)(T)(cst[2 + t] - Da * da[t]);
                        y0n = (double)(T)(cst[0] - lam * Da * da[AS]);
                    };
                    asm volatile("s_waitcnt lgkmcnt(0)" ::: "memory");
                    __builtin_amdgcn_wave_barrier();
                    int le[8];
#pragma unroll
                    for (int t = 0; t < 8; ++t) {
                        const unsigned w = clq[t >> 1];
                        le[t] = (int)(short)((t & 1) ? (w >> 16) : (w & 0xffffu));
                    }
                    double g0 = tot[0], h0 = tot[1];
#pragma unroll
                    for (int t = 0; t < 8; ++t)
                        if (le[t] >= 0 && (le[t] >> 8) == 0) {
                            g0 += sh_ce[(le[t] & 0xff) * 2];
                            h0 += sh_ce[(le[t] & 0xff) * 2 + 1];
                        }
                    double cc0[M + 1];
#pragma unroll
                    for (int t = 0; t <= M; ++t) cc0[t] = cache[t];
                    double dl = 0.0, res = pl;
                    for (int round = 0; round <= ncols + 1; ++round) {
                        if (lane < nc) {
                            double a1[AS], y0n;
                            after_a(sh_delta[qa], a1, y0n);
                            const double dAb = grad_factor<M>(a1, xb, pb);
                            sh_cv[lane * 2] = dloss_dev(LOSS, y0n, cst[1]) * dAb;
                            sh_cv[lane * 2 + 1] = dAb * dAb;
                        }
                        asm volatile("s_waitcnt lgkmcnt(0)" ::: "memory");
                        __builtin_amdgcn_wave_barrier();
                        double gq = g0, hq = h0;
#pragma unroll
                        for (int t = 0; t < 8; ++t)
                            if (le[t] >= 0 && (le[t] >> 8) != 0) {
                                gq += sh_cv[(le[t] & 0xff) * 2];
                                hq += sh_cv[(le[t] & 0xff) * 2 + 1];
                            }
#pragma unroll
                        for (int t = 0; t <= M; ++t) cache[t] = cc0[t];
                        res = pcd_chain_lanes<M>(reg, lane, ncols - 1, valid, pl, gq, hq, lam, mu,
                                                 beta, gamma, eta, cache, sh_chain);
                        const double dn = valid ? (pl - res) : 0.0;
                        const bool same = __double_as_longlong(dn) == __double_as_longlong(dl);
                        dl = dn;
                        sh_delta[lane] = dl;
                        asm volatile("s_waitcnt lgkmcnt(0)" ::: "memory");
                        __builtin_amdgcn_wave_barrier();
                        if (__ballot(!same) == 0ull) {
                            if (lane == 0 && g == a.G - 1) {
                                atomicAdd(&g_branch_count[BR_RELAX_STEPS], 1u);
                                atomicAdd(&g_branch_count[BR_RELAX_ROUNDS], (unsigned)(round + 1));
                            }
                            break;
                        }
                    }
                    if (g == 0 && valid) {
                        ps[jl] = res;
                        viol_pos[c0 + lane] = fabs(dl);
                    }
                    if (lane < nc && cfc.row / a.rows_per == g) {
                        const int i = cfc.row;
                        const double Db = sh_delta[qb];
                        double a1[AS], y0n;
                        after_a(sh_delta[qa], a1, y0n);
                        T a2[AS];
                        double db = xb;
#pragma unroll
                        for (int t = 0; t < AS; ++t) {
                            const double dn = xb * (a1[t] - pb * db);
                            a2[t] = (T)(a1[t] - Db * db);
                            db = dn;
                        }
                        const T y0f = (T)(y0n - lam * Db * db);
                        if constexpr (LDSR) {
#pragma unroll
                            for (int t = 0; t < AS; ++t) lds_a[(i - row0) * AS + t] = a2[t];
                            lds_r[i - row0] = y0f;
                        } else if constexpr (PK) {
                            float4 o;
                            o.x = (float)y0f;
                            o.y = (float)cst[1];
                            o.z = (float)a2[0];
                            o.w = (float)a2[AS - 1];
                            rec[(size_t)i] = o;
                        } else {
#pragma unroll
                            for (int t = 0; t < AS; ++t) A[(size_t)i * AS + t] = a2[t];
                            yy[2 * (size_t)i] = y0f;
                        }
                    }
                }
            }
            PRB_STAMP(4)
        }
        asm volatile("s_waitcnt lgkmcnt(0)\n\ts_barrier" ::: "memory");
        PRB_STAMP(5)
        PRB_WSTAMP(5)
        if (slot < ncols) {
            const double upd = sh_delta[slot];
            if (upd != 0.0) {
                const double p_old = sh_pold[slot];
#pragma unroll
                for (int u = 0; u < PRB_PF; ++u) {
                    if (cur.e0 + sub + 4 * u < cur.e1) {
                        const size_t i = (size_t)cur.row[u];
                        const double x = (double)cur.x[u];
                        if constexpr (M == 0) {
                            double yn = yh[u] - lam * av[u][0];
                            double an = av[u][0] / (1.0 + x * p_old);
                            an *= 1.0 + x * (p_old - upd);
                            yn += lam * an;
                            if constexpr (LDSR) {
                                lds_a[i - row0] = (T)an;
                                lds_r[i - row0] = (T)yn;
                            } else {
                                A[i] = (T)an;
                                yy[2 * i] = (T)yn;
                            }
                        } else if constexpr (LDSR) {
                            const int il = (int)i - row0;
                            double dprev = x;
#pragma unroll
                            for (int t = 0; t < AS; ++t) {
                                const double a1 = av[u][t];
                                const double dcur = x * (a1 - p_old * dprev);
                                lds_a[il * AS + t] = (T)(a1 - upd * dprev);
                                dprev = dcur;
                            }
                            lds_r[il] = (T)(yh[u] - lam * upd * dlast[u]);
                        } else if constexpr (PK) {
                            const double d1 = x * (av[u][0] - p_old * x);
                            float4 o;
                            o.x = (float)(yh[u] - lam * upd * dlast[u]);
                            o.y = (float)yt[u];
                            o.z = (float)(av[u][0] - upd * x);
                            o.w = (float)(av[u][AS - 1] - upd * d1);
                            rec[i] = o;
                        } else {
                            double dprev = x;
#pragma unroll
                            for (int t = 1; t < M; ++t) {
                                const double a1 = av[u][t - 1];
                                const double dcur = x * (a1 - p_old * dprev);
                                A[i * (M - 1) + (t - 1)] = (T)(a1 - upd * dprev);
                                dprev = dcur;
                            }
                            yy[2 * i] = (T)(yh[u] - lam * upd * dlast[u]);
                        }
                    }
                }
                for (int e = cur.e0 + sub + 4 * PRB_PF; e < cur.e1; e += 4) {
                    if constexpr (LDSR)
                        pcd_sync_entry_lds<T, M>(a.erow[e] - row0, (double)eval[e], p_old, upd,
                                                 lam, lds_a, lds_r);
                    else if constexpr (PK)
                        pcd_sync_entry_rec((size_t)a.erow[e], (double)eval[e], p_old, upd, lam, rec);
                    else
                        pcd_sync_entry<T, M>((size_t)a.erow[e], (double)eval[e], p_old, upd, lam,
                                             A, yy);
                }
            }
        }
        if (lmu != 0ull && worker) {
            const int32_t* spb = a.sp + ((size_t)g * a.nb + b) * 65;
            for (unsigned long long mm = lmu; mm != 0ull; mm &= mm - 1) {
                const int q = __builtin_ctzll(mm);
                const double upd = sh_delta[q];
                if (upd != 0.0) {
                    const double p_old = sh_pold[q];
                    const int le0 = spb[q], le1 = spb[q + 1];
                    for (int e = le0 + wt; e < le1; e += 256) {
                        if constexpr (LDSR)
                            pcd_sync_entry_lds<T, M>(a.erow[e] - row0, (double)eval[e], p_old,
                                                     upd, lam, lds_a, lds_r);
                        else if constexpr (PK)
                            pcd_sync_entry_rec((size_t)a.erow[e], (double)eval[e], p_old, upd, lam,
                                               rec);
                        else
                            pcd_sync_entry<T, M>((size_t)a.erow[e], (double)eval[e], p_old, upd,
                                                 lam, A, yy);
                    }
                }
            }
        }
        cur = nxt;
        p_slot = p_next;
        ne0 = n2e0;
        ne1 = n2e1;
        lm0 = lm1;
        lm1 = lm2;
        if constexpr (CR) {
            if (control) {
                cp0 = cp1;
                cp1 = cp2;
                cp2 = cp3;
                cp3 = a.cf_ptr[min(b + 4, a.nb)];
                cfc = cfn;
                clq = clqn;
            }
        }
        c0 = c1;
        c1 = c2;
        c2 = c3;
        c3 = c4;
        PRB_WSTAMP(6)
        if constexpr (LDSR)
            asm volatile("s_waitcnt lgkmcnt(0)\n\ts_barrier" ::: "memory");
        else
            __syncthreads();
        PRB_STAMP(6)
        if constexpr (STAMP) {
            if (tid == 320) tprev = clock64();
        }
        PRB_WSTAMP(7)
    }
#undef PRB_STAMP
#undef PRB_HSTAMP
#undef PRB_WSTAMP
    if constexpr (LDSR) {
        __syncthreads();
        const int nr = min(a.rows_per, a.n_rows - row0);
        for (int il = tid; il < nr; il += kPrbThreads) {
            const size_t i = (size_t)(row0 + il);
#pragma unroll
            for (int t = 0; t < AS; ++t) A[i * AS + t] = lds_a[il * AS + t];
            if constexpr (LR == 1)
                yy[2 * i] = (T)((double)lds_r[il] + (double)yy[2 * i + 1]);
            else
                yy[2 * i] = lds_r[il];
        }
    }
    if (STAMP && a.stamps != nullptr && (tid == 0 || tid == 64)) {
#pragma unroll
        for (int q = 0; q < 8; ++q)
            if (tid == 64 || (q != 1 && q != 2 && q != 7))
                a.stamps[(size_t)g * 16 + (tid == 64 ? 8 : 0) + q] = acc[q];
    }
    if (STAMP && a.stamps != nullptr && tid == 320) {
        a.stamps[(size_t)g * 16 + 1] = acc[1];
        a.stamps[(size_t)g * 16 + 2] = acc[2];
        a.stamps[(size_t)g * 16 + 7] = acc[7];
    }
}

template <typename T, int LOSS, int LR, bool MG = false, bool CR = false>
__global__ __launch_bounds__(kPrbThreads) void lin_prb_kernel(
    PrbArgs a, const T* __restrict__ eval, T* __restrict__ yy,
    const double* __restrict__ w_sched, const double* __restrict__ cn_sched,
    double* __restrict__ w, double alpha, double mu, double* __restrict__ viol_pos) {
    extern __shared__ __attribute__((aligned(16))) double dyn_lds[];
    double* sh_delta = dyn_lds + 128;
    double* sh_quart = dyn_lds + 1536;
    int* sh_ok = reinterpret_cast<int*>(dyn_lds + 768);
    int* sh_go = reinterpret_cast<int*>(dyn_lds + 770);
    const typename Vec2<T>::type* yy2 = reinterpret_cast<const typename Vec2<T>::type*>(yy);
    const int g = blockIdx.x;
    const int tid = threadIdx.x, lane = tid & 63, wave = tid >> 6;
    const bool control = wave == 0;
    const bool worker = wave >= 1 && wave <= 4;
    const int part = worker ? wave - 1 : (control ? 4 : wave);
    const int wt = tid - 64;
    const int slot = worker ? (wt >> 2) : 64, sub = wt & 3;
    double* sh_long = dyn_lds + 1024;
    static_assert(LR == 0 || (sizeof(T) == 4 && (LR == 2 || LOSS == LOSS_SQUARED)),
                  "LDS-resident rows: float storage");
    const int row0 = LR ? g * a.rows_per : 0;
    static_assert(!CR || !MG, "relaxed runs: single GPU");
    double* sh_ce = dyn_lds + kPrbLdsFixed;
    double* sh_cv = sh_ce + 64;
    T* lds_r = reinterpret_cast<T*>(dyn_lds + kPrbLdsFixed + (CR ? kPrbLdsCR : 0));
    unsigned char* lds_s = reinterpret_cast<unsigned char*>(lds_r + a.rows_per);
    if constexpr (LR != 0) {
        const int nr = min(a.rows_per, a.n_rows - row0);
        for (int il = tid; il < nr; il += kPrbThreads) {
            const typename Vec2<T>::type yv = yy2[(size_t)(row0 + il)];
            if constexpr (LR == 1) {
                lds_r[il] = (T)((double)yv.x - (double)yv.y);
            } else {
                lds_r[il] = yv.x;
                lds_s[il] = yv.y > (T)0 ? 1 : 0;
            }
        }
        __syncthreads();
    }
    auto row_state = [&](int i, double& y0, double& y1) {
        if constexpr (LR != 0) {
            y0 = (double)lds_r[i - row0];
            y1 = (LR == 1) ? 0.0 : (lds_s[i - row0] ? 1.0 : -1.0);
        } else {
            const typename Vec2<T>::type yv = yy2[(size_t)i];
            y0 = (double)yv.x;
            y1 = (double)yv.y;
        }
    };
    auto row_update = [&](int i, double yold, double dec) {
        if constexpr (LR != 0) lds_r[i - row0] = (T)(yold - dec);
        else yy[2 * (size_t)i] = (T)(yold - dec);
    };
    PrbEntries<T> cur, nxt;
    int c0 = a.bptr[0], c1 = a.bptr[1];
    int c2 = (a.nb > 1) ? a.bptr[2] : c1;
    int c3 = (a.nb > 2) ? a.bptr[3] : c2;
    unsigned long long lm0 = 0ull, lm1 = 0ull;
    {
        int e0, e1;
        prb_load_sp(a, g, 0, slot, c1 - c0, e0, e1, lm0);
        prb_load_entries<T>(a, eval, e0, e1, sub, cur, row0);
    }
    int ne0 = 0, ne1 = 0;
    if (a.nb > 1) prb_load_sp(a, g, 1, slot, c2 - c1, ne0, ne1, lm1);
    if (tid == 0) {
        *sh_ok = 1;
        *sh_go = 0;
    }
    int cp0 = 0, cp1 = 0, cp2 = 0, cp3 = 0;
    PrbConf<T> cfc, cfn;
    cfc.row = cfn.row = 0;
    cfc.qq = cfn.qq = 0;
    cfc.xa = cfc.xb = cfn.xa = cfn.xb = (T)0;
    prb_u4 clq = {~0u, ~0u, ~0u, ~0u}, clqn = {~0u, ~0u, ~0u, ~0u};
    if constexpr (CR) {
        if (control) {
            const PrbConf<T>* cfa = reinterpret_cast<const PrbConf<T>*>(a.cf);
            cp0 = a.cf_ptr[0];
            cp1 = a.cf_ptr[min(1, a.nb)];
            cp2 = a.cf_ptr[min(2, a.nb)];
            cp3 = a.cf_ptr[min(3, a.nb)];
            if (lane < cp1 - cp0) cfc = cfa[cp0 + lane];
            if (lane < c1 - c0) clq = reinterpret_cast<const prb_u4*>(a.clist)[c0 + lane];
        }
    }
    for (int b = 0; b < a.nb; ++b) {
        const int ncols = c1 - c0;
        const int c4 = (b + 4 <= a.nb) ? a.bptr[b + 4] : c3;
        double yh[PRB_PF];
        double wl = 0.0, cnl = 0.0;
        int jl = 0;
        double cst[2] = {0.0, 0.0};
        int n2e0 = 0, n2e1 = 0;
        unsigned long long lm2 = 0ull;
        const unsigned long long lmu =
            ((unsigned long long)__builtin_amdgcn_readfirstlane((int)(lm0 >> 32)) << 32) |
            (unsigned)__builtin_amdgcn_readfirstlane((int)lm0);
        if (lmu != 0ull) {
            const int32_t* spb = a.sp + ((size_t)g * a.nb + b) * 65;
            int qi = 0;
            for (unsigned long long mm = lmu; mm != 0ull; mm &= mm - 1, ++qi) {
                const int q = __builtin_ctzll(mm);
                if (worker) {
                    const int le0 = spb[q], le1 = spb[q + 1];
                    double lg = 0.0;
                    for (int e = le0 + wt; e < le1; e += 256) {
                        double y0, y1;
                        row_state(a.erow[e], y0, y1);
                        lg += dloss_dev(LOSS, y0, y1) * (double)eval[e];
                    }
                    lg = wave_sum(lg);
                    if (lane == 0) sh_long[(qi * 4 + (wave - 1)) * 2] = lg;
                }
            }
            __syncthreads();
            if (worker && wt < qi) {
                const int q = nth_set_bit(lmu, wt);
                double tg = 0.0;
                for (int w4 = 0; w4 < 4; ++w4) tg += sh_long[(wt * 4 + w4) * 2];
                double* sl = a.slab + (size_t)(b & 1) * a.G * 64 * 2 + ((size_t)g * 64 + q) * 2;
                prb_store_granule(sl, tg, prb_tag(b));
            }
        }
        if (control) {
            if (lane < ncols) {
                wl = w_sched[c0 + lane];
                cnl = cn_sched[c0 + lane];
                if (g == 0) jl = a.desc[c0 + lane].j;
            }
            if constexpr (CR) {
                const int nc = cp1 - cp0, ncw = max(nc, cp3 - cp2);
                const unsigned long long ctag = prb_tag(b);
                double* cs = a.cslab + ((size_t)(b & 1) * 64 + lane) * 8;
                if (lane < nc) {
                    if (cfc.row / a.rows_per == g) {
                        double y0, y1;
                        row_state(cfc.row, y0, y1);
                        prb_store_granule(cs, y0, ctag);
                        prb_store_granule(cs + 1, y1, ctag);
                    }
                } else if (lane < ncw && (lane % a.G) == g) {
                    prb_store_granule(cs, 0.0, ctag);
                    prb_store_granule(cs + 1, 0.0, ctag);
                }
            }
        } else if (worker) {
            double yt[PRB_PF];
#pragma unroll
            for (int u = 0; u < PRB_PF; ++u) row_state(cur.row[u], yh[u], yt[u]);
            double ag = 0.0;
#pragma unroll
            for (int u = 0; u < PRB_PF; ++u) {
                const bool v = cur.e0 + sub + 4 * u < cur.e1;
                ag += v ? dloss_dev(LOSS, yh[u], yt[u]) * (double)cur.x[u] : 0.0;
            }
            for (int e = cur.e0 + sub + 4 * PRB_PF; e < cur.e1; e += 4) {
                double y0, y1;
                row_state(a.erow[e], y0, y1);
                ag += dloss_dev(LOSS, y0, y1) * (double)eval[e];
            }
            ag += dpp_move_d<0xB1, 0xf>(0.0, ag);
            ag += dpp_move_d<0x4E, 0xf>(0.0, ag);
            if (sub == 0 && !((lm0 >> slot) & 1ull)) {
                double* sl = a.slab + (size_t)(b & 1) * a.G * 64 * 2 + ((size_t)g * 64 + slot) * 2;
                prb_store_granule(sl, ag, prb_tag(b));
            }
            if (tid == 64 + 255)
                __hip_atomic_store(sh_go, b + 1, __ATOMIC_RELAXED, __HIP_MEMORY_SCOPE_WORKGROUP);
            if (b + 2 < a.nb) prb_load_sp(a, g, b + 2, slot, c3 - c2, n2e0, n2e1, lm2);
            {
                const bool ok =
                    prb_collect_quarter<1>(a, b, part, lane, ncols, sh_quart, kPrbParts);
                if (!ok) *sh_ok = 0;
            }
            if (b + 1 < a.nb) {
                prb_load_entries<T>(a, eval, ne0, ne1, sub, nxt, row0);
            }
        } else if (!control) {
            if (b + 2 < a.nb) prb_load_sp(a, g, b + 2, slot, c3 - c2, n2e0, n2e1, lm2);
            unsigned spins = 0;
            while (__hip_atomic_load(sh_go, __ATOMIC_RELAXED, __HIP_MEMORY_SCOPE_WORKGROUP) <
                       b + 1 &&
                   ++spins < (1u << 24))
                __builtin_amdgcn_s_sleep(1);
            const bool ok = prb_collect_quarter<1>(a, b, part, lane, ncols, sh_quart, kPrbParts);
            if (!ok) *sh_ok = 0;
        }
        if (control) {
            if (b + 2 < a.nb) prb_load_sp(a, g, b + 2, slot, c3 - c2, n2e0, n2e1, lm2);
            {
                unsigned spins = 0;
                while (__hip_atomic_load(sh_go, __ATOMIC_RELAXED, __HIP_MEMORY_SCOPE_WORKGROUP) <
                           b + 1 &&
                       ++spins < (1u << 24))
                    __builtin_amdgcn_s_sleep(1);
                const bool ok =
                    prb_collect_quarter<1>(a, b, part, lane, ncols, sh_quart, kPrbParts);
                if (!ok) *sh_ok = 0;
            }
            if constexpr (CR) {
                if (lane < cp1 - cp0) {
                    if (!prb_poll<2>(a, a.cslab + ((size_t)(b & 1) * 64 + lane) * 8, prb_tag(b), cst))
                        *sh_ok = 0;
                }
                const PrbConf<T>* cfa = reinterpret_cast<const PrbConf<T>*>(a.cf);
                if (lane < cp2 - cp1) cfn = cfa[cp1 + lane];
                clqn = prb_u4{~0u, ~0u, ~0u, ~0u};
                if (lane < c2 - c1) clqn = reinterpret_cast<const prb_u4*>(a.clist)[c1 + lane];
            }
        }
        asm volatile("s_waitcnt lgkmcnt(0)\n\ts_barrier" ::: "memory");
        if (!*sh_ok) break;
        if (control) {
            double tot = sh_quart[lane * 2];
#pragma unroll
            for (int w = 1; w < kPrbParts; ++w) tot += sh_quart[(w * 64 + lane) * 2];
            if constexpr (MG) {
                if (!prb_cross_gpu<1>(a, g, b, lane, &tot)) *sh_ok = 0;
            }
            const bool valid = lane < ncols;
            bool relaxed_step = false;
            if constexpr (CR) relaxed_step = (cp1 - cp0) > 0;
            const double inv = mu * cnl + alpha;
            double upd = 0.0;
            if (!relaxed_step) {
                upd = tot;
                upd += alpha * wl;
                upd /= inv;
                if (!valid) upd = 0.0;
                sh_delta[lane] = upd;
            }
            if constexpr (CR) {
                if (relaxed_step) {
                    const int nc = cp1 - cp0;
                    const int qa = cfc.qq & 0xff, qb = cfc.qq >> 8;
                    const double xa = (double)cfc.xa, xb = (double)cfc.xb;
                    sh_delta[lane] = 0.0;
                    if (lane < nc) sh_ce[lane] = dloss_dev(LOSS, cst[0], cst[1]) * xa;
                    asm volatile("s_waitcnt lgkmcnt(0)" ::: "memory");
                    __builtin_amdgcn_wave_barrier();
                    int le[8];
#pragma unroll
                    for (int t = 0; t < 8; ++t) {
                        const unsigned wv = clq[t >> 1];
                        le[t] = (int)(short)((t & 1) ? (wv >> 16) : (wv & 0xffffu));
                    }
                    double g0 = tot;
#pragma unroll
                    for (int t = 0; t < 8; ++t)
                        if (le[t] >= 0 && (le[t] >> 8) == 0) g0 += sh_ce[le[t] & 0xff];
                    for (int round = 0; round <= ncols + 1; ++round) {
                        if (lane < nc) {
                            const double y0n = (double)(T)(cst[0] - sh_delta[qa] * xa);
                            sh_cv[lane] = dloss_dev(LOSS, y0n, cst[1]) * xb;
                        }
                        asm volatile("s_waitcnt lgkmcnt(0)" ::: "memory");
                        __builtin_amdgcn_wave_barrier();
                        double gq = g0;
#pragma unroll
                        for (int t = 0; t < 8; ++t)
                            if (le[t] >= 0 && (le[t] >> 8) != 0) gq += sh_cv[le[t] & 0xff];
                        double un = gq;
                        un += alpha * wl;
                        un /= inv;
                        if (!valid) un = 0.0;
                        const bool same = __double_as_longlong(un) == __double_as_longlong(upd);
                        upd = un;
                        sh_delta[lane] = upd;
                        asm volatile("s_waitcnt lgkmcnt(0)" ::: "memory");
                        __builtin_amdgcn_wave_barrier();
                        if (__ballot(!same) == 0ull) break;
                    }
                    if (lane < nc && cfc.row / a.rows_per == g) {
                        const double y0n = (double)(T)(cst[0] - sh_delta[qa] * xa);
                        row_update(cfc.row, y0n, sh_delta[qb] * xb);
                    }
                }
            }
            if (g == 0 && valid) {
                w[jl] = wl - upd;
                viol_pos[c0 + lane] = fabs(upd);
            }
        }
        asm volatile("s_waitcnt lgkmcnt(0)\n\ts_barrier" ::: "memory");
        if (slot < ncols) {
            const double upd = sh_delta[slot];
            if (upd != 0.0) {
#pragma unroll
                for (int u = 0; u < PRB_PF; ++u)
                    if (cur.e0 + sub + 4 * u < cur.e1)
                        row_update(cur.row[u], yh[u], upd * (double)cur.x[u]);
                for (int e = cur.e0 + sub + 4 * PRB_PF; e < cur.e1; e += 4) {
                    double y0, y1;
                    row_state(a.erow[e], y0, y1);
                    row_update(a.erow[e], y0, upd * (double)eval[e]);
                }
            }
        }
        if (lmu != 0ull && worker) {
            const int32_t* spb = a.sp + ((size_t)g * a.nb + b) * 65;
            for (unsigned long long mm = lmu; mm != 0ull; mm &= mm - 1) {
                const int q = __builtin_ctzll(mm);
                const double upd = sh_delta[q];
                if (upd != 0.0) {
                    const int le0 = spb[q], le1 = spb[q + 1];
                    for (int e = le0 + wt; e < le1; e += 256) {
                        double y0, y1;
                        row_state(a.erow[e], y0, y1);
                        row_update(a.erow[e], y0, upd * (double)eval[e]);
                    }
                }
            }
        }
        cur = nxt;
        ne0 = n2e0;
        ne1 = n2e1;
        lm0 = lm1;
        lm1 = lm2;
        if constexpr (CR) {
            if (control) {
                cp0 = cp1;
                cp1 = cp2;
                cp2 = cp3;
                cp3 = a.cf_ptr[min(b + 4, a.nb)];
                cfc = cfn;
                clq = clqn;
            }
        }
        c0 = c1;
        c1 = c2;
        c2 = c3;
        c3 = c4;
        if constexpr (LR != 0)
            asm volatile("s_waitcnt lgkmcnt(0)\n\ts_barrier" ::: "memory");
        else
            __syncthreads();
    }
    if constexpr (LR != 0) {
        __syncthreads();
        const int nr = min(a.rows_per, a.n_rows - row0);
        for (int il = tid; il < nr; il += kPrbThreads) {
            const size_t i = (size_t)(row0 + il);
            if constexpr (LR == 1)
                yy[2 * i] = (T)((double)lds_r[il] + (double)yy[2 * i + 1]);
            else
                yy[2 * i] = lds_r[il];
        }
    }
}

static __global__ __launch_bounds__(kWave) void hop_pingpong_kernel(unsigned long long* words,
                                                             int rounds, int partner,
                                                             int* info ) {
    const int b = blockIdx.x;
    if ((b != 0 && b != partner) || threadIdx.x != 0) return;
    const int me = (b == 0) ? 0 : 1;
    info[me] = (int)__builtin_amdgcn_s_getreg((3 << 11) | 20);
    unsigned long long* mine = words + (me ? 16 : 0);
    unsigned long long* theirs = words + (me ? 0 : 16);
    for (int r = 1; r <= rounds; ++r) {
        if (me == 0)
            __hip_atomic_store(mine, (unsigned long long)r, __ATOMIC_RELAXED,
                               __HIP_MEMORY_SCOPE_AGENT);
        unsigned spins = 0;
        while (__hip_atomic_load(theirs, __ATOMIC_RELAXED, __HIP_MEMORY_SCOPE_AGENT) <
               (unsigned long long)r) {
            if (++spins > (1u << 22)) {
                info[2] = r;
                return;
            }
        }
        if (me == 1)
            __hip_atomic_store(mine, (unsigned long long)r, __ATOMIC_RELAXED,
                               __HIP_MEMORY_SCOPE_AGENT);
    }
}

template <int NV>
__device__ __forceinline__ bool prb_poll(const PrbArgs& a, const double* p,
                                         unsigned long long tag, double* out) {
    unsigned long long t[NV];
    unsigned spins = 0;
    for (;;) {
        bool all = true;
#pragma unroll
        for (int v = 0; v < NV; ++v) {
            t[v] = prb_load_granule(p + v);
            all = all && ((t[v] & 3ull) == tag);
        }
        if (all) break;
        if ((++spins & 63u) == 0) {
            if (__hip_atomic_load(a.abort_flag, __ATOMIC_RELAXED, __HIP_MEMORY_SCOPE_AGENT) ||
                spins > a.spin_max) {
                __hip_atomic_store(a.abort_flag, 1u, __ATOMIC_RELAXED, __HIP_MEMORY_SCOPE_AGENT);
                return false;
            }
        }
    }
#pragma unroll
    for (int v = 0; v < NV; ++v) out[v] = __longlong_as_double((long long)(t[v] & ~3ull));
    return true;
}

static __global__ __launch_bounds__(768) void exchange_probe_kernel(PrbArgs a, int rounds,
                                                                     int ncols, int readers_mod,
                                                                     int xcd_mode) {
    __shared__ double quart[8 * 64 * 2];
    __shared__ int ok_flag;
    __shared__ int go_flag;
    __shared__ int my_rank;
    int g = blockIdx.x;
    if (xcd_mode) {
        if (threadIdx.x == 0) {
            const int xcc = (int)__builtin_amdgcn_s_getreg((3 << 11) | 20);
            int r = -1;
            if (xcc == xcd_mode - 1) r = (int)atomicAdd(a.abort_flag + 1, 1u);
            my_rank = (r >= 0 && r < a.G) ? r : -1;
        }
        __syncthreads();
        g = my_rank;
        if (g < 0) return;
    }
    const int tid = threadIdx.x, lane = tid & 63, wave = tid >> 6;
    const bool control = wave == 0;
    const int wt = tid - 64, slot = (wave >= 1 && wave <= 4) ? (wt >> 2) : 64, sub = wt & 3;
    const bool eight = readers_mod < 0;
    if (eight) readers_mod = 1;
    const bool sweeps = (g % readers_mod) == 0;
    if (tid == 0) {
        ok_flag = 1;
        go_flag = 0;
    }
    __syncthreads();
    for (int b = 0; b < rounds; ++b) {
        const unsigned long long tag = prb_tag(b);
        if (eight) {
            const bool worker = wave >= 1 && wave <= 4;
            if (worker) {
                if (sub == 0) {
                    double* sl =
                        a.slab + (size_t)(b & 1) * a.G * 64 * 2 + ((size_t)g * 64 + slot) * 2;
                    if (xcd_mode) {
                        prb_store_granule_l2(sl, 1.0 + b, tag);
                        prb_store_granule_l2(sl + 1, 2.0 + g, tag);
                    } else {
                        prb_store_granule(sl, 1.0 + b, tag);
                        prb_store_granule(sl + 1, 2.0 + g, tag);
                    }
                }
                if (tid == 64 + 255)
                    __hip_atomic_store(&go_flag, b + 1, __ATOMIC_RELAXED,
                                       __HIP_MEMORY_SCOPE_WORKGROUP);
            } else {
                unsigned spins = 0;
                while (__hip_atomic_load(&go_flag, __ATOMIC_RELAXED, __HIP_MEMORY_SCOPE_WORKGROUP) <
                           b + 1 &&
                       ++spins < (1u << 24))
                    __builtin_amdgcn_s_sleep(1);
            }
            if (blockDim.x == 768) {
                if (!worker) {
                    const int part12 = control ? 0 : wave - 4;
                    if (!prb_collect_quarter<2>(a, b, part12, lane, ncols, quart, 8)) ok_flag = 0;
                }
            } else {
                const int part = worker ? wave - 1 : (control ? 4 : wave);
                if (!prb_collect_quarter<2>(a, b, part, lane, ncols, quart, 8)) ok_flag = 0;
            }
            __syncthreads();
            if (!ok_flag) break;
            continue;
        }
        if (!control && wave <= 4) {
            if (sub == 0) {
                double* sl = a.slab + (size_t)(b & 1) * a.G * 64 * 2 + ((size_t)g * 64 + slot) * 2;
                prb_store_granule(sl, 1.0 + b, tag);
                prb_store_granule(sl + 1, 2.0 + g, tag);
            }
            if (sweeps && !prb_collect_quarter<2>(a, b, wave - 1, lane, ncols, quart)) ok_flag = 0;
        }
        __syncthreads();
        if (!ok_flag) break;
        if (readers_mod > 1 && control) {
            double* tb = a.slab + (size_t)2 * a.G * 64 * 2 +
                         ((size_t)(b & 1) * a.G + (g / readers_mod)) * 64 * 2 + (size_t)lane * 2;
            if (sweeps) {
                prb_store_granule(tb, quart[lane * 2], tag);
                prb_store_granule(tb + 1, quart[lane * 2 + 1], tag);
            } else {
                double t2[2];
                bool okp = true;
                if (lane < ncols) okp = prb_poll<2>(a, tb, tag, t2);
                if (!__all(okp)) ok_flag = 0;
            }
        }
        __syncthreads();
        if (!ok_flag) break;
    }
}

static __global__ __launch_bounds__(kWave) void peer_probe_kernel(double* const* slabs, size_t off,
                                                           int n_ranks, int rank,
                                                           unsigned long long word,
                                                           unsigned long long max_ticks, int* ok) {
    const int r = threadIdx.x;
    bool good = true;
    if (r < n_ranks) {
        __hip_atomic_store(reinterpret_cast<unsigned long long*>(slabs[r] + off) + rank, word,
                           __ATOMIC_RELAXED, __HIP_MEMORY_SCOPE_SYSTEM);
        const unsigned long long* mine =
            reinterpret_cast<const unsigned long long*>(slabs[rank] + off) + r;
        const unsigned long long t0 = wall_clock64();
        while (__hip_atomic_load(mine, __ATOMIC_RELAXED, __HIP_MEMORY_SCOPE_SYSTEM) != word) {
            if (wall_clock64() - t0 > max_ticks) {
                good = false;
                break;
            }
            __builtin_amdgcn_s_sleep(8);
        }
    }
    const bool all = __all(good);
    if (threadIdx.x == 0) ok[0] = all ? 1 : 0;
}

template <typename T>
__global__ __launch_bounds__(kPrbThreads) void prb_stream_probe_kernel(PrbArgs a,
                                                                      const T* __restrict__ eval,
                                                                      double* __restrict__ sink) {
    const int g = blockIdx.x, tid = threadIdx.x, wave = tid >> 6;
    const bool worker = wave >= 1 && wave <= 4;
    const int wt = tid - 64, slot = worker ? (wt >> 2) : 64, sub = wt & 3;
    double acc = 0.0;
    for (int b = 0; b < a.nb; ++b) {
        const int ncols = a.bptr[b + 1] - a.bptr[b];
        int e0, e1;
        unsigned long long lm;
        prb_load_sp(a, g, b, slot, ncols, e0, e1, lm);
        for (int e = e0 + sub; e < e1; e += 4) acc += (double)a.erow[e] + (double)eval[e];
    }
    sink[(size_t)g * kPrbThreads + tid] = acc;
}

template <int BYTES>
__global__ __launch_bounds__(kPrbThreads) void prb_write_probe_kernel(PrbArgs a,
                                                                     float* __restrict__ records) {
    static_assert(BYTES == 4 || BYTES == 8 || BYTES == 16, "record width");
    const int g = blockIdx.x, tid = threadIdx.x, wave = tid >> 6;
    const bool worker = wave >= 1 && wave <= 4;
    const int wt = tid - 64, slot = worker ? (wt >> 2) : 64, sub = wt & 3;
    for (int b = 0; b < a.nb; ++b) {
        const int ncols = a.bptr[b + 1] - a.bptr[b];
        int e0, e1;
        unsigned long long lm;
        prb_load_sp(a, g, b, slot, ncols, e0, e1, lm);
        for (int e = e0 + sub; e < e1; e += 4) {
            const size_t row = (size_t)a.erow[e];
            const float v = (float)(b + e);
            if constexpr (BYTES == 4) records[row] = v;
            else if constexpr (BYTES == 8) reinterpret_cast<float2*>(records)[row] = make_float2(v, v);
            else reinterpret_cast<float4*>(records)[row] = make_float4(v, v, v, v);
        }
    }
}

static __global__ void gather_sched_kernel(int d, const ColDesc* __restrict__ desc,
                                    const double* __restrict__ v, double* __restrict__ out) {
    const int pos = blockIdx.x * blockDim.x + threadIdx.x;
    if (pos < d) out[pos] = v[desc[pos].j];
}

static __global__ void fold_viol_kernel(int d, const ColDesc* __restrict__ desc,
                                 const double* __restrict__ viol_pos,
                                 double* __restrict__ viol_col) {
    const int pos = blockIdx.x * blockDim.x + threadIdx.x;
    if (pos < d) viol_col[desc[pos].j] += viol_pos[pos];
}

static __global__ void snapshot_row_kernel(const Ctl* __restrict__ ctl, const double* __restrict__ P,
                                    int d, const ColDesc* __restrict__ desc,
                                    double* __restrict__ out) {
    const int pos = blockIdx.x * blockDim.x + threadIdx.x;
    if (pos < d) out[pos] = P[(size_t)ctl->s * d + desc[pos].j];
}

template <typename T>
__global__ void prb_gather_kernel(int64_t nnz, const int32_t* __restrict__ src,
                                  const int32_t* __restrict__ cidx, const T* __restrict__ cval,
                                  int32_t* __restrict__ erow, T* __restrict__ eval) {
    const int64_t e = (int64_t)blockIdx.x * blockDim.x + threadIdx.x;
    if (e < nnz) {
        const int32_t q = src[e];
        erow[e] = cidx[q];
        eval[e] = cval[q];
    }
}


}
```

sparsepoly_amd/engine.py:

```python
import collections
import contextlib
import ctypes as C
import threading

import numpy as np
import scipy.sparse as sp

from . import _capi


class SpfmError(RuntimeError):
    pass


def canonical_csc(X):
    if sp.issparse(X):
        Xc = sp.csc_matrix(X, dtype=np.float64, copy=True)
        Xc.sum_duplicates()
        Xc.sort_indices()
    else:
        Xc = sp.csc_matrix(np.asarray(X, dtype=np.float64))
        Xc.sort_indices()
    return Xc

# ... 341 lines not shown

    @contextlib.contextmanager
    def _interaction_features(self, n_features):
        if n_features is None or n_features >= self.d:
            yield
            return
        old = self.get_option("interaction_features")
        self.set_option("interaction_features", int(n_features))
        try:
            yield
        finally:
            self.set_option("interaction_features", old)

    def release_interaction_scratch(self):
        self.set_option("interaction_release", 1)

    def interaction_stats(self, order_idx, tol=0.0, n_features=None):
        with self._interaction_features(n_features):
            return self._interaction_stats(order_idx, tol)

    def _interaction_stats(self, order_idx, tol):
        cnt = np.zeros(2, dtype=np.int64)
        sums = np.zeros(3)
        self._check(self._lib.spfm_interaction_stats(
            self._h, int(order_idx), float(tol), cnt.ctypes.data_as(_capi._lp),
            sums.ctypes.data_as(_capi._dp)))
        return dict(nnz=int(cnt[0]), active_features=int(cnt[1]), sum_sq=float(sums[0]),
                    sum_abs=float(sums[1]), max_abs=float(sums[2]))

    def interaction_topk(self, order_idx, K, n_features=None):
        with self._interaction_features(n_features):
            return self._interaction_topk(order_idx, K)

    def _interaction_topk(self, order_idx, K):
        K = int(K)
        rows = np.zeros(max(K, 1), dtype=np.int32)
        cols = np.zeros(max(K, 1), dtype=np.int32)
        vals = np.zeros(max(K, 1))
        n = C.c_int64()
        self._check(self._lib.spfm_interaction_topk(
            self._h, int(order_idx), K, rows.ctypes.data_as(_capi._ip),
            cols.ctypes.data_as(_capi._ip), vals.ctypes.data_as(_capi._dp), C.byref(n)))
        return rows[:n.value].copy(), cols[:n.value].copy(), vals[:n.value].copy()

    def interaction_list(self, order_idx, tol, capacity, n_features=None):
        with self._interaction_features(n_features):
            return self._interaction_list(order_idx, tol, capacity)

    def _interaction_list(self, order_idx, tol, capacity):
        capacity = int(capacity)
        rows = np.zeros(max(capacity, 1), dtype=np.int32)
        cols = np.zeros(max(capacity, 1), dtype=np.int32)
        vals = np.zeros(max(capacity, 1))
        n = C.c_int64()
        self._check(self._lib.spfm_interaction_list(
            self._h, int(order_idx), float(tol), capacity, rows.ctypes.data_as(_capi._ip),
            cols.ctypes.data_as(_capi._ip), vals.ctypes.data_as(_capi._dp), C.byref(n)))
        return rows[:n.value].copy(), cols[:n.value].copy(), vals[:n.value].copy()

    def interaction_values(self, order_idx, rows, cols):
        ra, rp = _capi.i32(rows)
        ca, cp = _capi.i32(cols)
        if ra.ndim != 1 or ra.shape != ca.shape:
            raise ValueError("rows and cols must be 1-d arrays of one length")
        vals = np.zeros(ra.shape[0])
        self._check(self._lib.spfm_interaction_values(
            self._h, int(order_idx), ra.shape[0], rp, cp, vals.ctypes.data_as(_capi._dp)))
        return vals

    def interaction_block(self, order_idx, J, J2=None):
        ja, jp = _capi.i32(J)
        j2a, j2p = (ja, jp) if J2 is None else _capi.i32(J2)
        if ja.ndim != 1 or j2a.ndim != 1:
            raise ValueError("J and J2 must be 1-d index arrays")
        if ja.shape[0] * j2a.shape[0] * 8 > _capi.INTERACTION_BLOCK_MAX_BYTES:
            raise ValueError("interaction_block: %d x %d doubles exceed the budget of %d bytes"
                             % (ja.shape[0], j2a.shape[0], _capi.INTERACTION_BLOCK_MAX_BYTES))
        out = np.zeros((ja.shape[0], j2a.shape[0]))
        self._check(self._lib.spfm_interaction_block(
            self._h, int(order_idx), ja.shape[0], jp, j2a.shape[0], j2p,
            out.ctypes.data_as(_capi._dp)))
        return out

    def set_schedule(self, mode, indices_feature, conflict_csc=None):
        jf, jp = _capi.i32(indices_feature)
        order = np.empty(self.d, dtype=np.int32)
        nb = C.c_int32()
        if conflict_csc is None:
            cp, ci, rows = None, None, 0
        else:
            cpa, cp = _capi.i64(conflict_csc.indptr)
            cia, ci = _capi.i32(conflict_csc.indices)
            rows = conflict_csc.shape[0]
        self._check(self._lib.spfm_set_schedule(
            self._h, _capi.SCHEDULES[mode], jp, cp, ci, rows,
            order.ctypes.data_as(_capi._ip), C.byref(nb)))
        self.order, self.n_batches = order, nb.value
        return order

    def get_schedule(self, mode="colored"):
        from .schedule import Schedule

        nb = C.c_int32()
        self._check(self._lib.spfm_get_schedule(self._h, None, None, C.byref(nb)))
        order = np.empty(self.d, dtype=np.int32)
        bp = np.empty(nb.value + 1, dtype=np.int32)
        self._check(self._lib.spfm_get_schedule(self._h, order.ctypes.data_as(_capi._ip),
                                                bp.ctypes.data_as(_capi._ip), C.byref(nb)))
        return Schedule(order, bp, mode, (self.n, self.d))

    def install_schedule(self, sched, conflict_csc=None):
        oa, op = _capi.i32(sched.order)
        ba, bp = _capi.i32(sched.batch_ptr)
        if oa.shape[0] != self.d:
            raise ValueError("schedule has %d features, the data has %d" % (oa.shape[0], self.d))
        if conflict_csc is None:
            cp, ci, rows = None, None, 0
        else:
            cpa, cp = _capi.i64(conflict_csc.indptr)
            cia, ci = _capi.i32(conflict_csc.indices)
            rows = conflict_csc.shape[0]
        self._check(self._lib.spfm_set_schedule_raw(self._h, op, bp, ba.shape[0] - 1, cp, ci,
                                                    rows))
        self.order, self.n_batches = oa.copy(), ba.shape[0] - 1
        return self.order

    def cd_linear_epoch(self, alpha):
        v = C.c_double()
        self._check(self._lib.spfm_cd_linear_epoch(self._h, float(alpha), C.byref(v)))
        return v.value

    def pcd_epoch(self, order_idx, degree, beta, gamma, eta, indices_component):
        ic, icp = _capi.i32(indices_component)
        v = C.c_double()
        self._check(self._lib.spfm_pcd_epoch(
            self._h, int(order_idx), int(degree), float(beta), float(gamma), float(eta), icp,
            ic.shape[0], C.byref(v)))
        return v.value

    def pbcd_epoch(self, order_idx, degree, beta, gamma, eta):
        v = C.c_double()
        self._check(self._lib.spfm_pbcd_epoch(
            self._h, int(order_idx), int(degree), float(beta), float(gamma), float(eta),
            C.byref(v)))
        return v.value

    _MU = {"squared": 1.0, "logistic": 0.25, "squared_hinge": 2.0}

    def _host_steps(self):
        sched = self.get_schedule()
        return sched.order, sched.batch_ptr

    def pcd_epoch_host(self, reg, P, lams, loss, order_idx, degree, beta, gamma, eta,
                       indices_component):
        mu = self._MU[loss]
        order, bp = self._host_steps()
        self._check(self._lib.spfm_host_epoch_begin(self._h, int(order_idx), int(degree)))
        reg.compute_cache_pcd_all(P, degree)
        viol = 0.0
        sums = np.empty((int(np.diff(bp).max()), 2))
        for s in indices_component:
            s = int(s)
            self._check(self._lib.spfm_host_pass_begin(self._h, s))
            reg.compute_cache_pcd(P, degree, s)
            for b in range(len(bp) - 1):
                cols = order[bp[b]:bp[b + 1]]
                nc = len(cols)
                if nc == 0:
                    continue
                self._check(self._lib.spfm_host_step_sums(self._h, b,
                                                          sums.ctypes.data_as(_capi._dp)))
                p_new = np.empty(nc)
                for q in range(nc):
                    j = int(cols[q])
                    p_old = float(P[s, j])
                    inv = mu * sums[q, 1] + beta
                    upd = (lams[s] * sums[q, 0] + beta * p_old) / inv
                    pn = float(reg.prox_cd(p_old - eta * upd, eta * gamma / inv, degree, j))
                    viol += abs(p_old - pn)
                    P[s, j] = pn
                    p_new[q] = pn
                    reg.update_cache_pcd(P, degree, s, j)
                self._check(self._lib.spfm_host_step_apply(
                    self._h, b, p_new.ctypes.data_as(_capi._dp), None))
        dv = C.c_double()
        self._check(self._lib.spfm_host_epoch_end(self._h, C.byref(dv)))
        return viol

    def pbcd_epoch_host(self, reg, Pt, lams, loss, order_idx, degree, beta, gamma, eta):
        mu = self._MU[loss]
        order, bp = self._host_steps()
        k = Pt.shape[1]
        lams = np.asarray(lams, dtype=np.float64)
        self._check(self._lib.spfm_host_epoch_begin(self._h, int(order_idx), int(degree)))
        reg.compute_cache_pbcd(Pt, degree)
        viol = 0.0
        sums = np.empty((int(np.diff(bp).max()), k + 1))
        for b in range(len(bp) - 1):
            cols = order[bp[b]:bp[b + 1]]
            nc = len(cols)
            if nc == 0:
                continue
            self._check(self._lib.spfm_host_step_sums(self._h, b, sums.ctypes.data_as(_capi._dp)))
            p_new = np.empty((nc, k))
            p_old = np.empty((nc, k))
            for q in range(nc):
                j = int(cols[q])
                p_old[q] = Pt[j]
                inv = mu * sums[q, k] + beta
                grad = (sums[q, :k] * lams + beta * Pt[j]) / inv
                pj = Pt[j] - eta * grad
                reg.prox_bcd(pj, eta * gamma / inv, degree, j)
                viol += float(np.abs(p_old[q] - pj).sum())
                Pt[j] = pj
                p_new[q] = pj
                reg.update_cache_pbcd(Pt, degree, j)
            self._check(self._lib.spfm_host_step_apply(
                self._h, b, p_new.ctypes.data_as(_capi._dp), p_old.ctypes.data_as(_capi._dp)))
        dv = C.c_double()
        self._check(self._lib.spfm_host_epoch_end(self._h, C.byref(dv)))
        return viol

    def psgd_epoch(self, degree, alpha, beta, gamma, eta0, learning_rate, power_t, batch_size,
                   indices_samples, fit_linear, it, row_lo=None):
        idx = np.ascontiguousarray(indices_samples, dtype=np.int32)
        itc = C.c_int64(int(it))
        sl = C.c_double()
        lr = (_capi.LEARNING_RATE[learning_rate] if isinstance(learning_rate, str)
              else int(learning_rate))
        if row_lo is not None:
            self._check(self._lib.spfm_psgd_epoch_sharded(
                self._h, int(degree), float(alpha), float(beta), float(gamma), float(eta0), lr,
                float(power_t), int(batch_size), idx.ctypes.data_as(_capi._ip), idx.size,
                int(row_lo), int(bool(fit_linear)), C.byref(itc), C.byref(sl)))
            return sl.value, itc.value
        self._check(self._lib.spfm_psgd_epoch(
            self._h, int(degree), float(alpha), float(beta), float(gamma), float(eta0), lr,
            float(power_t), int(batch_size), idx.ctypes.data_as(_capi._ip), idx.size,
            int(bool(fit_linear)), C.byref(itc), C.byref(sl)))
        return sl.value, itc.value

    @staticmethod
    def comm_unique_id():
        lib = _capi.load()
        buf = C.create_string_buffer(128)
        rc = lib.spfm_comm_unique_id(buf)
        if rc != 0:
            raise SpfmError("spfm_comm_unique_id: %s" % lib.spfm_last_error(None).decode())
        return buf.raw

    def comm_init(self, uid, n_ranks, rank):
        assert len(uid) == 128
        self._check(self._lib.spfm_comm_init(self._h, uid, int(n_ranks), int(rank)))

    def comm_init_shm(self, name, n_ranks, rank):
        self._check(self._lib.spfm_comm_init_shm(self._h, name.encode(), int(n_ranks), int(rank)))

    def peer_alloc(self):
        buf = C.create_string_buffer(64)
        self._check(self._lib.spfm_peer_alloc(self._h, buf))
        return buf.raw

    def peer_connect(self, n_ranks, rank, handles):
        blob = b"".join(handles)
        assert len(blob) == 64 * n_ranks
        self._check(self._lib.spfm_peer_connect(self._h, int(n_ranks), int(rank), blob))

    def profile_enable(self, on=True):
        self._check(self._lib.spfm_profile_enable(self._h, int(bool(on))))

    def profile_reset(self):
        self._check(self._lib.spfm_profile_reset(self._h))

    def profile_get(self, which):
        ms, nl, nz = C.c_double(), C.c_int64(), C.c_int64()
        self._check(self._lib.spfm_profile_get(self._h, int(which), C.byref(ms), C.byref(nl),
                                               C.byref(nz)))
        return ms.value, nl.value, nz.value

    def set_use_graph(self, on):
        self._check(self._lib.spfm_set_use_graph(self._h, int(bool(on))))

    def debug_hop_latency(self, partner=1, rounds=20000):
        ns = C.c_double()
        xcc = (C.c_int32 * 2)()
        self._check(self._lib.spfm_debug_hop_latency(self._h, int(partner), int(rounds),
                                                     C.byref(ns), xcc))
        return ns.value, (xcc[0], xcc[1])

    def debug_exchange_cost(self, groups=64, ncols=37, readers_mod=1, rounds=5000):
        ns = C.c_double()
        self._check(self._lib.spfm_debug_exchange_cost(self._h, int(groups), int(ncols),
                                                       int(readers_mod), int(rounds),
                                                       C.byref(ns)))
        return ns.value

    def debug_prb_stamps(self):
        buf = np.zeros(16 * 512, dtype=np.int64)
        nv = self._lib.spfm_debug_prb_stamps(self._h, buf.ctypes.data_as(_capi._lp), buf.size)
        if nv < 0:
            self._check(nv)
        return buf[:nv].reshape(-1, 16)

    def debug_branch_counts(self, reset=True):
        buf = (C.c_uint32 * 8)()
        self._check(self._lib.spfm_debug_branch_counts(self._h, buf, int(bool(reset))))
        return dict(omegati_clip=buf[0], omegacs_dcache=buf[1], omegacs_cache=buf[2],
                    squaredl21_resum=buf[3], relax_steps=buf[4], relax_rounds=buf[5])

    def debug_stream_probe(self):
        nb = C.c_int64()
        self._check(self._lib.spfm_debug_stream_probe(self._h, C.byref(nb)))
        return nb.value

    def debug_write_probe(self, bytes_per_record):
        nb = C.c_int64()
        self._check(self._lib.spfm_debug_write_probe(self._h, int(bytes_per_record), C.byref(nb)))
        return nb.value

    def get_option(self, key):
        v = C.c_int()
        self._check(self._lib.spfm_get_option(self._h, key.encode(), C.byref(v)))
        return v.value

    def set_option(self, key, value):
        self._check(self._lib.spfm_set_option(self._h, key.encode(), int(value)))
```

Before: 3.697 epochs/s.

## Register-cache extra column entries, pack LDS row state, unroll image load/writeback

```diff
diff --git a/sparsepoly_amd/csrc/spfm_engine_core.hip b/sparsepoly_amd/csrc/spfm_engine_core.hip
--- a/sparsepoly_amd/csrc/spfm_engine_core.hip
+++ b/sparsepoly_amd/csrc/spfm_engine_core.hip
@@ -1394,7 +1394,8 @@
     if (!h->prb_ready || !out) return SPFM_ERR_INVALID;
     const int nval = 16 * h->prb_G;
     if (cap < nval) return SPFM_ERR_INVALID;
-    if (hipMemcpy(out, h->prb_stamps.p, sizeof(long long) * (size_t)nval, hipMemcpyDeviceToHost) !=
+    const int ncopy = (cap >= nval + 4 * h->prb_G) ? nval + 4 * h->prb_G : nval;
+    if (hipMemcpy(out, h->prb_stamps.p, sizeof(long long) * (size_t)ncopy, hipMemcpyDeviceToHost) !=
         hipSuccess)
         return SPFM_ERR_RUNTIME;
     return nval;
diff --git a/sparsepoly_amd/csrc/spfm_engine_prb.inc.h b/sparsepoly_amd/csrc/spfm_engine_prb.inc.h
--- a/sparsepoly_amd/csrc/spfm_engine_prb.inc.h
+++ b/sparsepoly_amd/csrc/spfm_engine_prb.inc.h
@@ -156,7 +156,7 @@
     HIPC(prow_old.alloc(sizeof(double) * (size_t)d));
     HIPC(prb_viol.alloc(sizeof(double) * (size_t)d));
     HIPC(prb_cn.alloc(sizeof(double) * (size_t)d));
-    HIPC(prb_stamps.alloc(sizeof(long long) * 16 * (size_t)prb_G));
+    HIPC(prb_stamps.alloc(sizeof(long long) * (16 + 4) * (size_t)prb_G));
     HIPC(hipMemsetAsync(prb_stamps.p, 0, prb_stamps.bytes, stream));
     HIPC(hipMemsetAsync(prb_abort.p, 0, sizeof(unsigned) * 4, stream));
     HIPC(hipMemsetAsync(prb_slab.p, 0, prb_slab.bytes, stream));
diff --git a/sparsepoly_amd/csrc/spfm_pcd.hip.h b/sparsepoly_amd/csrc/spfm_pcd.hip.h
--- a/sparsepoly_amd/csrc/spfm_pcd.hip.h
+++ b/sparsepoly_amd/csrc/spfm_pcd.hip.h
@@ -699,16 +699,28 @@
 __device__ __forceinline__ void pcd_sync_entry_lds(int il, double x, double p_old, double upd,
                                                    double lam, T* lds_a, T* lds_r) {
     constexpr int AS = Kind<M>::AS;
-    double yh = (double)lds_r[il];
-    if constexpr (M == 0) {
-        const double a0 = (double)lds_a[il];
-        yh -= lam * a0;
-        double a1 = a0 / (1.0 + x * p_old);
-        a1 *= 1.0 + x * (p_old - upd);
-        yh += lam * a1;
-        lds_a[il] = (T)a1;
-        lds_r[il] = (T)yh;
+    if constexpr (AS == 1) {
+        using P2 = typename Vec2<T>::type;
+        P2* lds_p = reinterpret_cast<P2*>(lds_a);
+        const P2 pr = lds_p[il];
+        const double a0 = (double)pr.x;
+        double yh = (double)pr.y;
+        P2 o;
+        if constexpr (M == 0) {
+            yh -= lam * a0;
+            double a1 = a0 / (1.0 + x * p_old);
+            a1 *= 1.0 + x * (p_old - upd);
+            yh += lam * a1;
+            o.x = (T)a1;
+            o.y = (T)yh;
+        } else {
+            const double d1 = x * (a0 - p_old * x);
+            o.x = (T)(a0 - upd * x);
+            o.y = (T)(yh - lam * upd * d1);
+        }
+        lds_p[il] = o;
     } else {
+        double yh = (double)lds_r[il];
         double dprev = x;
 #pragma unroll
         for (int t = 0; t < AS; ++t) {
diff --git a/sparsepoly_amd/csrc/spfm_prb.hip.h b/sparsepoly_amd/csrc/spfm_prb.hip.h
--- a/sparsepoly_amd/csrc/spfm_prb.hip.h
+++ b/sparsepoly_amd/csrc/spfm_prb.hip.h
@@ -211,13 +211,27 @@
 }
 
 constexpr int PRB_PF = 4;
+constexpr int PRB_PX = 2;
 constexpr int kPrbLong = 48;
 template <typename T>
 struct PrbEntries {
     int e0, e1;
     int row[PRB_PF];
     T x[PRB_PF];
+    int rowx[PRB_PX];
+    T xx[PRB_PX];
 };
+template <typename T>
+__device__ __forceinline__ void prb_clear_extras(PrbEntries<T>& en, int pad_row) {
+#pragma unroll
+    for (int u = 0; u < PRB_PX; ++u) {
+        en.rowx[u] = pad_row;
+        en.xx[u] = (T)0;
+    }
+}
+__device__ __forceinline__ bool prb_wave_has_extras(int e0, int e1, int sub) {
+    return __ballot(e0 + sub + 4 * PRB_PF < e1) != 0ull;
+}
 
 __device__ __forceinline__ void prb_load_sp(const PrbArgs& a, int g, int b, int slot, int ncols,
                                             int& e0, int& e1, unsigned long long& lmask) {
@@ -243,7 +257,7 @@
     return __builtin_ctzll(m);
 }
 
-template <typename T>
+template <typename T, bool XTRA = true>
 __device__ __forceinline__ void prb_load_entries(const PrbArgs& a, const T* __restrict__ eval,
                                                  int e0, int e1, int sub, PrbEntries<T>& en,
                                                  int pad_row = 0) {
@@ -256,10 +270,20 @@
         en.row[u] = v ? a.erow[e] : pad_row;
         en.x[u] = v ? eval[e] : (T)0;
     }
+    if (XTRA && prb_wave_has_extras(e0, e1, sub)) {
+#pragma unroll
+        for (int u = 0; u < PRB_PX; ++u) {
+            const int e = e0 + sub + 4 * (PRB_PF + u);
+            const bool v = e < e1;
+            en.rowx[u] = v ? a.erow[e] : pad_row;
+            en.xx[u] = v ? eval[e] : (T)0;
+        }
+    }
 }
 
 constexpr int kPrbThreads = 512;
 constexpr int kPrbParts = 8;
+constexpr int kPrbImgU = 8;
 constexpr int kPrbLdsFixed = 2560;
 
 template <int NV>
@@ -357,22 +381,90 @@
     T* lds_a = reinterpret_cast<T*>(dyn_lds + kPrbLdsFixed + (CR ? kPrbLdsCR : 0));
     T* lds_r = lds_a + (size_t)a.rows_per * AS;
     unsigned char* lds_s = reinterpret_cast<unsigned char*>(lds_r + a.rows_per);
+    constexpr bool PAIR = LDSR && AS == 1;
+    constexpr bool XTRA = AS == 1 || (AS == 2 && !CR);
+    constexpr int NREG = PRB_PF + (XTRA ? PRB_PX : 0);
+    using P2 = typename Vec2<T>::type;
+    P2* lds_p = reinterpret_cast<P2*>(lds_a);
+    auto lds_get = [&](int il, double* av_, double& yh_) __attribute__((always_inline)) {
+        if constexpr (PAIR) {
+            const P2 pr = lds_p[il];
+            av_[0] = (double)pr.x;
+            yh_ = (double)pr.y;
+        } else {
+            yh_ = (double)lds_r[il];
+#pragma unroll
+            for (int t = 0; t < AS; ++t) av_[t] = (double)lds_a[il * AS + t];
+        }
+    };
+    auto lds_put = [&](int il, const T* an_, T yn_) __attribute__((always_inline)) {
+        if constexpr (PAIR) {
+            P2 pr;
+            pr.x = an_[0];
+            pr.y = yn_;
+            lds_p[il] = pr;
+        } else {
+#pragma unroll
+            for (int t = 0; t < AS; ++t) lds_a[il * AS + t] = an_[t];
+            lds_r[il] = yn_;
+        }
+    };
+    auto gather_row = [&](int i, double* av_, double& yh_, double& yt_) __attribute__((always_inline)) {
+        if constexpr (LDSR) {
+            lds_get(i - row0, av_, yh_);
+            yt_ = (LR == 1) ? 0.0 : (lds_s[i - row0] ? 1.0 : -1.0);
+        } else if constexpr (PK) {
+            const float4 r = rec[(size_t)i];
+            yh_ = (double)r.x;
+            yt_ = (double)r.y;
+            av_[0] = (double)r.z;
+            av_[AS - 1] = (double)r.w;
+        } else {
+            const typename Vec2<T>::type yv = yy2[(size_t)i];
+            yh_ = (double)yv.x;
+            yt_ = (double)yv.y;
+#pragma unroll
+            for (int t = 0; t < AS; ++t) av_[t] = (double)A[(size_t)i * AS + t];
+        }
+    };
+    int* sh_over = reinterpret_cast<int*>(dyn_lds + 772);
+    if constexpr (STAMP) {
+        if (tid == 0) sh_over[0] = sh_over[1] = 0;
+        __syncthreads();
+    }
+    const long long t_img = STAMP ? clock64() : 0;
+    long long x_img = 0, x_wb = 0, n_over16 = 0, n_over24 = 0;
     if constexpr (LDSR) {
         const int nr = min(a.rows_per, a.n_rows - row0);
-        for (int il = tid; il < nr; il += kPrbThreads) {
-            const typename Vec2<T>::type yv = yy2[(size_t)(row0 + il)];
-#pragma unroll
-            for (int t = 0; t < AS; ++t) lds_a[il * AS + t] = A[(size_t)(row0 + il) * AS + t];
-            if constexpr (LR == 1) {
-                lds_r[il] = (T)((double)yv.x - (double)yv.y);
-            } else {
-                lds_r[il] = yv.x;
-                lds_s[il] = yv.y > (T)0 ? 1 : 0;
+        for (int il0 = tid; il0 < nr; il0 += kPrbImgU * kPrbThreads) {
+            typename Vec2<T>::type yv[kPrbImgU];
+            T an[kPrbImgU][AS];
+#pragma unroll
+            for (int u = 0; u < kPrbImgU; ++u) {
+                const int il = min(il0 + u * kPrbThreads, nr - 1);
+                yv[u] = yy2[(size_t)(row0 + il)];
+#pragma unroll
+                for (int t = 0; t < AS; ++t) an[u][t] = A[(size_t)(row0 + il) * AS + t];
+            }
+#pragma unroll
+            for (int u = 0; u < kPrbImgU; ++u) {
+                const int il = il0 + u * kPrbThreads;
+                if (il < nr) {
+                    if constexpr (LR == 1) {
+                        lds_put(il, an[u], (T)((double)yv[u].x - (double)yv[u].y));
+                    } else {
+                        lds_put(il, an[u], yv[u].x);
+                        lds_s[il] = yv[u].y > (T)0 ? 1 : 0;
+                    }
+                }
             }
         }
         __syncthreads();
     }
+    if constexpr (STAMP) x_img = clock64() - t_img;
     PrbEntries<T> cur, nxt;
+    prb_clear_extras(cur, row0);
+    prb_clear_extras(nxt, row0);
     int c0 = a.bptr[0], c1 = a.bptr[1];
     int c2 = (a.nb > 1) ? a.bptr[2] : c1;
     int c3 = (a.nb > 2) ? a.bptr[3] : c2;
@@ -380,7 +472,7 @@
     {
         int e0, e1;
         prb_load_sp(a, g, 0, slot, c1 - c0, e0, e1, lm0);
-        prb_load_entries<T>(a, eval, e0, e1, sub, cur, row0);
+        prb_load_entries<T, XTRA>(a, eval, e0, e1, sub, cur, row0);
     }
     int ne0 = 0, ne1 = 0;
     if (a.nb > 1) prb_load_sp(a, g, 1, slot, c2 - c1, ne0, ne1, lm1);
@@ -440,6 +532,9 @@
         __builtin_amdgcn_s_waitcnt(0x0F70);
         double av[PRB_PF][AS];
         double yh[PRB_PF], yt[PRB_PF], dlast[PRB_PF];
+        double avx[PRB_PX][AS];
+        double yhx[PRB_PX], ytx[PRB_PX], dlastx[PRB_PX];
+        bool wx = false;
         double pl = 0.0;
         int jl = 0;
         double cst[CSN];
@@ -458,24 +553,7 @@
                     const int i = cfc.row;
                     if (i / a.rows_per == g) {
                         double st[CSN];
-                        if constexpr (LDSR) {
-                            st[0] = (double)lds_r[i - row0];
-                            st[1] = (LR == 1) ? 0.0 : (lds_s[i - row0] ? 1.0 : -1.0);
-#pragma unroll
-                            for (int t = 0; t < AS; ++t) st[2 + t] = (double)lds_a[(i - row0) * AS + t];
-                        } else if constexpr (PK) {
-                            const float4 r = rec[(size_t)i];
-                            st[0] = (double)r.x;
-                            st[1] = (double)r.y;
-                            st[2] = (double)r.z;
-                            st[2 + AS - 1] = (double)r.w;
-                        } else {
-                            const typename Vec2<T>::type yv = yy2[(size_t)i];
-                            st[0] = (double)yv.x;
-                            st[1] = (double)yv.y;
-#pragma unroll
-                            for (int t = 0; t < AS; ++t) st[2 + t] = (double)A[(size_t)i * AS + t];
-                        }
+                        gather_row(i, st + 2, st[0], st[1]);
 #pragma unroll
                         for (int t = 0; t < CSN; ++t) prb_store_granule(cs + t, st[t], ctag);
                     }
@@ -486,28 +564,8 @@
             }
         } else if (worker) {
 #pragma unroll
-            for (int u = 0; u < PRB_PF; ++u) {
-                if constexpr (LDSR) {
-                    const int il = cur.row[u] - row0;
-                    yh[u] = (double)lds_r[il];
-                    yt[u] = (LR == 1) ? 0.0 : (lds_s[il] ? 1.0 : -1.0);
-#pragma unroll
-                    for (int t = 0; t < AS; ++t) av[u][t] = (double)lds_a[il * AS + t];
-                } else if constexpr (PK) {
-                    const float4 r = rec[(size_t)cur.row[u]];
-                    yh[u] = (double)r.x;
-                    yt[u] = (double)r.y;
-                    av[u][0] = (double)r.z;
-                    av[u][AS - 1] = (double)r.w;
-                } else {
-                    const size_t i = (size_t)cur.row[u];
-                    const typename Vec2<T>::type yv = yy2[i];
-                    yh[u] = (double)yv.x;
-                    yt[u] = (double)yv.y;
-#pragma unroll
-                    for (int t = 0; t < AS; ++t) av[u][t] = (double)A[i * AS + t];
-                }
-            }
+            for (int u = 0; u < PRB_PF; ++u)
+                gather_row(cur.row[u], av[u], yh[u], yt[u]);
             double ag = 0.0, ah = 0.0;
 #pragma unroll
             for (int u = 0; u < PRB_PF; ++u) {
@@ -518,28 +576,32 @@
                 ag += v ? dl * dprev : 0.0;
                 ah += v ? dprev * dprev : 0.0;
             }
-            for (int e = cur.e0 + sub + 4 * PRB_PF; e < cur.e1; e += 4) {
+            if constexpr (STAMP) {
+                const bool o16 = __ballot(cur.e0 + sub + 16 < cur.e1) != 0ull;
+                const bool o24 = __ballot(cur.e0 + sub + 24 < cur.e1) != 0ull;
+                if (lane == 0 && o16) atomicMax(&sh_over[0], b + 1);
+                if (lane == 0 && o24) atomicMax(&sh_over[1], b + 1);
+            }
+            wx = XTRA && prb_wave_has_extras(cur.e0, cur.e1, sub);
+            if (wx) {
+#pragma unroll
+                for (int u = 0; u < PRB_PX; ++u)
+                    gather_row(cur.rowx[u], avx[u], yhx[u], ytx[u]);
+#pragma unroll
+                for (int u = 0; u < PRB_PX; ++u) {
+                    const double dprev = grad_factor<M>(avx[u], (double)cur.xx[u], p_slot);
+                    dlastx[u] = dprev;
+                    const double dl = dloss_dev(LOSS, yhx[u], ytx[u]);
+                    const bool v = cur.e0 + sub + 4 * (PRB_PF + u) < cur.e1;
+                    ag += v ? dl * dprev : 0.0;
+                    ah += v ? dprev * dprev : 0.0;
+                }
+            }
+            for (int e = cur.e0 + sub + 4 * NREG; e < cur.e1; e += 4) {
                 const int i = a.erow[e];
                 const double x = (double)eval[e];
                 double a1[AS], y0, y1;
-                if constexpr (LDSR) {
-                    y0 = (double)lds_r[i - row0];
-                    y1 = (LR == 1) ? 0.0 : (lds_s[i - row0] ? 1.0 : -1.0);
-#pragma unroll
-                    for (int t = 0; t < AS; ++t) a1[t] = (double)lds_a[(i - row0) * AS + t];
-                } else if constexpr (PK) {
-                    const float4 r = rec[(size_t)i];
-                    y0 = (double)r.x;
-                    y1 = (double)r.y;
-                    a1[0] = (double)r.z;
-                    a1[AS - 1] = (double)r.w;
-                } else {
-                    const typename Vec2<T>::type yv = yy2[i];
-                    y0 = (double)yv.x;
-                    y1 = (double)yv.y;
-#pragma unroll
-                    for (int t = 0; t < AS; ++t) a1[t] = (double)A[(size_t)i * AS + t];
-                }
+                gather_row(i, a1, y0, y1);
                 const double dprev = grad_factor<M>(a1, x, p_slot);
                 ag += dloss_dev(LOSS, y0, y1) * dprev;
                 ah += dprev * dprev;
@@ -572,26 +634,7 @@
                         const int i = a.erow[e];
                         const double x = (double)eval[e];
                         double a1[Kind<M>::AS], y0, y1;
-                        if constexpr (LDSR) {
-                            y0 = (double)lds_r[i - row0];
-                            y1 = (LR == 1) ? 0.0 : (lds_s[i - row0] ? 1.0 : -1.0);
-#pragma unroll
-                            for (int t = 0; t < Kind<M>::AS; ++t)
-                                a1[t] = (double)lds_a[(i - row0) * Kind<M>::AS + t];
-                        } else if constexpr (PK) {
-                            const float4 r = rec[(size_t)i];
-                            y0 = (double)r.x;
-                            y1 = (double)r.y;
-                            a1[0] = (double)r.z;
-                            a1[Kind<M>::AS - 1] = (double)r.w;
-                        } else {
-                            const typename Vec2<T>::type yv = yy2[i];
-                            y0 = (double)yv.x;
-                            y1 = (double)yv.y;
-#pragma unroll
-                            for (int t = 0; t < Kind<M>::AS; ++t)
-                                a1[t] = (double)A[(size_t)i * Kind<M>::AS + t];
-                        }
+                        gather_row(i, a1, y0, y1);
                         const double dprev = grad_factor<M>(a1, x, pq);
                         lg += dloss_dev(LOSS, y0, y1) * dprev;
                         lh += dprev * dprev;
@@ -628,7 +671,7 @@
             if (tid == 64 + 255)
                 __hip_atomic_store(sh_go, b + 1, __ATOMIC_RELAXED, __HIP_MEMORY_SCOPE_WORKGROUP);
             if (LDSR && b + 1 < a.nb) {
-                prb_load_entries<T>(a, eval, ne0, ne1, sub, nxt, row0);
+                prb_load_entries<T, XTRA>(a, eval, ne0, ne1, sub, nxt, row0);
                 if (slot < c2 - c1) p_next = pold_sched[c1 + slot];
             }
             {
@@ -638,7 +681,7 @@
             }
             PRB_WSTAMP(2)
             if (!LDSR && b + 1 < a.nb) {
-                prb_load_entries<T>(a, eval, ne0, ne1, sub, nxt, row0);
+                prb_load_entries<T, XTRA>(a, eval, ne0, ne1, sub, nxt, row0);
                 if (slot < c2 - c1) p_next = pold_sched[c1 + slot];
             }
         } else {
@@ -668,6 +711,12 @@
         PRB_WSTAMP(3)
         asm volatile("s_waitcnt lgkmcnt(0)\n\ts_barrier" ::: "memory");
         if (!*sh_ok) break;
+        if constexpr (STAMP) {
+            if (tid == 0) {
+                n_over16 += sh_over[0] == b + 1;
+                n_over24 += sh_over[1] == b + 1;
+            }
+        }
         PRB_STAMP(3)
         PRB_HSTAMP(7)
         PRB_WSTAMP(4)
@@ -796,9 +845,7 @@
                         }
                         const T y0f = (T)(y0n - lam * Db * db);
                         if constexpr (LDSR) {
-#pragma unroll
-                            for (int t = 0; t < AS; ++t) lds_a[(i - row0) * AS + t] = a2[t];
-                            lds_r[i - row0] = y0f;
+                            lds_put(i - row0, a2, y0f);
                         } else if constexpr (PK) {
                             float4 o;
                             o.x = (float)y0f;
@@ -823,56 +870,72 @@
             const double upd = sh_delta[slot];
             if (upd != 0.0) {
                 const double p_old = sh_pold[slot];
-#pragma unroll
-                for (int u = 0; u < PRB_PF; ++u) {
-                    if (cur.e0 + sub + 4 * u < cur.e1) {
-                        const size_t i = (size_t)cur.row[u];
-                        const double x = (double)cur.x[u];
-                        if constexpr (M == 0) {
-                            double yn = yh[u] - lam * av[u][0];
-                            double an = av[u][0] / (1.0 + x * p_old);
-                            an *= 1.0 + x * (p_old - upd);
-                            yn += lam * an;
-                            if constexpr (LDSR) {
-                                lds_a[i - row0] = (T)an;
-                                lds_r[i - row0] = (T)yn;
+                auto scatter_row = [&](int row, double x, const double* av_, double yh_, double yt_,
+                                       double dlast_) __attribute__((always_inline)) {
+                    const size_t i = (size_t)row;
+                    if constexpr (M == 0) {
+                        double yn = yh_ - lam * av_[0];
+                        double an = av_[0] / (1.0 + x * p_old);
+                        an *= 1.0 + x * (p_old - upd);
+                        yn += lam * an;
+                        if constexpr (LDSR) {
+                            const T an_t[1] = {(T)an};
+                            lds_put(row - row0, an_t, (T)yn);
+                        } else {
+                            A[i] = (T)an;
+                            yy[2 * i] = (T)yn;
+                        }
+                    } else if constexpr (LDSR) {
+                        T an[AS];
+                        double dprev = x;
+#pragma unroll
+                        for (int t = 0; t < AS; ++t) {
+                            const double a1 = av_[t];
+                            const double dcur = x * (a1 - p_old * dprev);
+                            an[t] = (T)(a1 - upd * dprev);
+                            dprev = dcur;
+                        }
+                        lds_put(row - row0, an, (T)(yh_ - lam * upd * dlast_));
+                    } else if constexpr (PK) {
+                        const double d1 = x * (av_[0] - p_old * x);
+                        float4 o;
+                        o.x = (float)(yh_ - lam * upd * dlast_);
+                        o.y = (float)yt_;
+                        o.z = (float)(av_[0] - upd * x);
+                        o.w = (float)(av_[AS - 1] - upd * d1);
+                        rec[i] = o;
+                    } else {
+                        double dprev = x;
+#pragma unroll
+                        for (int t = 1; t < M; ++t) {
+                            const double a1 = av_[t - 1];
+                            const double dcur = x * (a1 - p_old * dprev);
+                            A[i * (M - 1) + (t - 1)] = (T)(a1 - upd * dprev);
+                            dprev = dcur;
+                        }
+                        yy[2 * i] = (T)(yh_ - lam * upd * dlast_);
+                    }
+                };
+#pragma unroll
+                for (int u = 0; u < PRB_PF; ++u)
+                    if (cur.e0 + sub + 4 * u < cur.e1)
+                        scatter_row(cur.row[u], (double)cur.x[u], av[u], yh[u], yt[u], dlast[u]);
+                if (wx) {
+#pragma unroll
+                    for (int u = 0; u < PRB_PX; ++u)
+                        if (cur.e0 + sub + 4 * (PRB_PF + u) < cur.e1) {
+                            if constexpr (AS == 1) {
+                                scatter_row(cur.rowx[u], (double)cur.xx[u], avx[u], yhx[u], ytx[u],
+                                            dlastx[u]);
                             } else {
-                                A[i] = (T)an;
-                                yy[2 * i] = (T)yn;
+                                double a1[AS], y0, y1;
+                                gather_row(cur.rowx[u], a1, y0, y1);
+                                scatter_row(cur.rowx[u], (double)cur.xx[u], a1, y0, y1,
+                                            grad_factor<M>(a1, (double)cur.xx[u], p_slot));
                             }
-                        } else if constexpr (LDSR) {
-                            const int il = (int)i - row0;
-                            double dprev = x;
-#pragma unroll
-                            for (int t = 0; t < AS; ++t) {
-                                const double a1 = av[u][t];
-                                const double dcur = x * (a1 - p_old * dprev);
-                                lds_a[il * AS + t] = (T)(a1 - upd * dprev);
-                                dprev = dcur;
-                            }
-                            lds_r[il] = (T)(yh[u] - lam * upd * dlast[u]);
-                        } else if constexpr (PK) {
-                            const double d1 = x * (av[u][0] - p_old * x);
-                            float4 o;
-                            o.x = (float)(yh[u] - lam * upd * dlast[u]);
-                            o.y = (float)yt[u];
-                            o.z = (float)(av[u][0] - upd * x);
-                            o.w = (float)(av[u][AS - 1] - upd * d1);
-                            rec[i] = o;
-                        } else {
-                            double dprev = x;
-#pragma unroll
-                            for (int t = 1; t < M; ++t) {
-                                const double a1 = av[u][t - 1];
-                                const double dcur = x * (a1 - p_old * dprev);
-                                A[i * (M - 1) + (t - 1)] = (T)(a1 - upd * dprev);
-                                dprev = dcur;
-                            }
-                            yy[2 * i] = (T)(yh[u] - lam * upd * dlast[u]);
                         }
-                    }
-                }
-                for (int e = cur.e0 + sub + 4 * PRB_PF; e < cur.e1; e += 4) {
+                }
+                for (int e = cur.e0 + sub + 4 * NREG; e < cur.e1; e += 4) {
                     if constexpr (LDSR)
                         pcd_sync_entry_lds<T, M>(a.erow[e] - row0, (double)eval[e], p_old, upd,
                                                  lam, lds_a, lds_r);
@@ -942,16 +1005,41 @@
 #undef PRB_WSTAMP
     if constexpr (LDSR) {
         __syncthreads();
+        const long long t_wb = STAMP ? clock64() : 0;
         const int nr = min(a.rows_per, a.n_rows - row0);
-        for (int il = tid; il < nr; il += kPrbThreads) {
-            const size_t i = (size_t)(row0 + il);
-#pragma unroll
-            for (int t = 0; t < AS; ++t) A[i * AS + t] = lds_a[il * AS + t];
-            if constexpr (LR == 1)
-                yy[2 * i] = (T)((double)lds_r[il] + (double)yy[2 * i + 1]);
-            else
-                yy[2 * i] = lds_r[il];
-        }
+        for (int il0 = tid; il0 < nr; il0 += kPrbImgU * kPrbThreads) {
+            double an[kPrbImgU][AS], yn[kPrbImgU], yt[kPrbImgU];
+#pragma unroll
+            for (int u = 0; u < kPrbImgU; ++u) {
+                const int il = min(il0 + u * kPrbThreads, nr - 1);
+                lds_get(il, an[u], yn[u]);
+                yt[u] = (LR == 1) ? (double)yy[2 * (size_t)(row0 + il) + 1] : 0.0;
+            }
+#pragma unroll
+            for (int u = 0; u < kPrbImgU; ++u) {
+                const int il = il0 + u * kPrbThreads;
+                if (il < nr) {
+                    const size_t i = (size_t)(row0 + il);
+#pragma unroll
+                    for (int t = 0; t < AS; ++t) A[i * AS + t] = (T)an[u][t];
+                    if constexpr (LR == 1)
+                        yy[2 * i] = (T)(yn[u] + yt[u]);
+                    else
+                        yy[2 * i] = (T)yn[u];
+                }
+            }
+        }
+        if constexpr (STAMP) {
+            __syncthreads();
+            x_wb = clock64() - t_wb;
+        }
+    }
+    if (STAMP && a.stamps != nullptr && tid == 0) {
+        long long* xs = a.stamps + (size_t)a.G * 16 + (size_t)g * 4;
+        xs[0] = n_over16;
+        xs[1] = n_over24;
+        xs[2] = x_img;
+        xs[3] = x_wb;
     }
     if (STAMP && a.stamps != nullptr && (tid == 0 || tid == 64)) {
 #pragma unroll
@@ -995,13 +1083,22 @@
     unsigned char* lds_s = reinterpret_cast<unsigned char*>(lds_r + a.rows_per);
     if constexpr (LR != 0) {
         const int nr = min(a.rows_per, a.n_rows - row0);
-        for (int il = tid; il < nr; il += kPrbThreads) {
-            const typename Vec2<T>::type yv = yy2[(size_t)(row0 + il)];
-            if constexpr (LR == 1) {
-                lds_r[il] = (T)((double)yv.x - (double)yv.y);
-            } else {
-                lds_r[il] = yv.x;
-                lds_s[il] = yv.y > (T)0 ? 1 : 0;
+        for (int il0 = tid; il0 < nr; il0 += kPrbImgU * kPrbThreads) {
+            typename Vec2<T>::type yv[kPrbImgU];
+#pragma unroll
+            for (int u = 0; u < kPrbImgU; ++u)
+                yv[u] = yy2[(size_t)(row0 + min(il0 + u * kPrbThreads, nr - 1))];
+#pragma unroll
+            for (int u = 0; u < kPrbImgU; ++u) {
+                const int il = il0 + u * kPrbThreads;
+                if (il < nr) {
+                    if constexpr (LR == 1) {
+                        lds_r[il] = (T)((double)yv[u].x - (double)yv[u].y);
+                    } else {
+                        lds_r[il] = yv[u].x;
+                        lds_s[il] = yv[u].y > (T)0 ? 1 : 0;
+                    }
+                }
             }
         }
         __syncthreads();
@@ -1021,6 +1118,8 @@
         else yy[2 * (size_t)i] = (T)(yold - dec);
     };
     PrbEntries<T> cur, nxt;
+    prb_clear_extras(cur, row0);
+    prb_clear_extras(nxt, row0);
     int c0 = a.bptr[0], c1 = a.bptr[1];
     int c2 = (a.nb > 1) ? a.bptr[2] : c1;
     int c3 = (a.nb > 2) ? a.bptr[3] : c2;
@@ -1057,6 +1156,8 @@
         const int ncols = c1 - c0;
         const int c4 = (b + 4 <= a.nb) ? a.bptr[b + 4] : c3;
         double yh[PRB_PF];
+        double yhx[PRB_PX];
+        bool wx = false;
         double wl = 0.0, cnl = 0.0;
         int jl = 0;
         double cst[2] = {0.0, 0.0};
@@ -1123,7 +1224,18 @@
                 const bool v = cur.e0 + sub + 4 * u < cur.e1;
                 ag += v ? dloss_dev(LOSS, yh[u], yt[u]) * (double)cur.x[u] : 0.0;
             }
-            for (int e = cur.e0 + sub + 4 * PRB_PF; e < cur.e1; e += 4) {
+            wx = prb_wave_has_extras(cur.e0, cur.e1, sub);
+            if (wx) {
+                double ytx[PRB_PX];
+#pragma unroll
+                for (int u = 0; u < PRB_PX; ++u) row_state(cur.rowx[u], yhx[u], ytx[u]);
+#pragma unroll
+                for (int u = 0; u < PRB_PX; ++u) {
+                    const bool v = cur.e0 + sub + 4 * (PRB_PF + u) < cur.e1;
+                    ag += v ? dloss_dev(LOSS, yhx[u], ytx[u]) * (double)cur.xx[u] : 0.0;
+                }
+            }
+            for (int e = cur.e0 + sub + 4 * (PRB_PF + PRB_PX); e < cur.e1; e += 4) {
                 double y0, y1;
                 row_state(a.erow[e], y0, y1);
                 ag += dloss_dev(LOSS, y0, y1) * (double)eval[e];
@@ -1259,7 +1371,13 @@
                 for (int u = 0; u < PRB_PF; ++u)
                     if (cur.e0 + sub + 4 * u < cur.e1)
                         row_update(cur.row[u], yh[u], upd * (double)cur.x[u]);
-                for (int e = cur.e0 + sub + 4 * PRB_PF; e < cur.e1; e += 4) {
+                if (wx) {
+#pragma unroll
+                    for (int u = 0; u < PRB_PX; ++u)
+                        if (cur.e0 + sub + 4 * (PRB_PF + u) < cur.e1)
+                            row_update(cur.rowx[u], yhx[u], upd * (double)cur.xx[u]);
+                }
+                for (int e = cur.e0 + sub + 4 * (PRB_PF + PRB_PX); e < cur.e1; e += 4) {
                     double y0, y1;
                     row_state(a.erow[e], y0, y1);
                     row_update(a.erow[e], y0, upd * (double)eval[e]);
@@ -1308,12 +1426,23 @@
     if constexpr (LR != 0) {
         __syncthreads();
         const int nr = min(a.rows_per, a.n_rows - row0);
-        for (int il = tid; il < nr; il += kPrbThreads) {
-            const size_t i = (size_t)(row0 + il);
-            if constexpr (LR == 1)
-                yy[2 * i] = (T)((double)lds_r[il] + (double)yy[2 * i + 1]);
-            else
-                yy[2 * i] = lds_r[il];
+        for (int il0 = tid; il0 < nr; il0 += kPrbImgU * kPrbThreads) {
+            double yt[kPrbImgU];
+#pragma unroll
+            for (int u = 0; u < kPrbImgU; ++u)
+                yt[u] = (LR == 1) ? (double)yy[2 * (size_t)(row0 + min(il0 + u * kPrbThreads, nr - 1)) + 1]
+                                  : 0.0;
+#pragma unroll
+            for (int u = 0; u < kPrbImgU; ++u) {
+                const int il = il0 + u * kPrbThreads;
+                if (il < nr) {
+                    const size_t i = (size_t)(row0 + il);
+                    if constexpr (LR == 1)
+                        yy[2 * i] = (T)((double)lds_r[il] + yt[u]);
+                    else
+                        yy[2 * i] = lds_r[il];
+                }
+            }
         }
     }
 }
diff --git a/sparsepoly_amd/engine.py b/sparsepoly_amd/engine.py
--- a/sparsepoly_amd/engine.py
+++ b/sparsepoly_amd/engine.py
@@ -667,6 +667,18 @@
             self._check(nv)
         return buf[:nv].reshape(-1, 16)
 
+    def debug_prb_slot_stamps(self):
+        buf = np.full(20 * 512, -1, dtype=np.int64)
+        nv = self._lib.spfm_debug_prb_stamps(self._h, buf.ctypes.data_as(_capi._lp), buf.size)
+        if nv < 0:
+            self._check(nv)
+        xs = buf[nv:nv + nv // 4]
+        if nv == 0 or nv % 16 or (xs < 0).any():
+            raise RuntimeError("spfm_debug_prb_stamps returned no slot values: they follow the "
+                               "timers of the 64-column pcd pass only (option prb_stamps, no "
+                               "pcdw_stamps / pbprb_stamps / pbprb_dbg)")
+        return xs.reshape(-1, 4)
+
     def debug_branch_counts(self, reset=True):
         buf = (C.c_uint32 * 8)()
         self._check(self._lib.spfm_debug_branch_counts(self._h, buf, int(bool(reset))))
```

Result: faster. 3.822 epochs/s (median of 6 runs) (+3.4%).
